# hermda02/dang

Measured on AMD Instinct MI355X. Metric: gibbs_iterations_per_sec, higher is better.
Workload: dtype f64

## Files before the change

### dang_amd/_lib.py

```python
import ctypes as C
import os

_HERE = os.path.dirname(os.path.abspath(__file__))
LIB_PATH = os.environ.get("DANGX_LIB") or os.path.join(_HERE, "lib", "libdangx.so")

MAX_BANDS, MAX_COMPS, MAX_IND, MAX_GROUP = 32, 16, 2, 8

POWERLAW, MBB, FREEFREE, LOGNORMAL, CMB, TCMB, TEMPLATE, MONOPOLE, HIFIT = 1, 2, 3, 4, 5, 6, 7, 8, 9
LNL_CHISQ, LNL_MARGINAL, LNL_PRIOR = 1, 2, 3
PRIOR_GAUSSIAN, PRIOR_UNIFORM, PRIOR_JEFFREYS = 1, 2, 3
ML_SAMPLE, ML_OPTIMIZE = 1, 2
FLAG_T, FLAG_Q, FLAG_U, FLAG_QU = 1, 2, 4, 8
SOLVER_DIRECT, SOLVER_CG = 0, 1
FLUCT_CORRECT, FLUCT_REFERENCE = 0, 1
COARSE_REFERENCE, COARSE_DEGRADED = 0, 1
COARSE_MODEL_CODES = {"reference": COARSE_REFERENCE, "degraded": COARSE_DEGRADED}
A2T, A2F, F2T = 0, 1, 2
UNIT_CODES = {"uK_RJ": 0, "uK_cmb": 1, "MJy/sr": 2}
K_AMP_DIRECT, K_INDEX_MH, K_SKY_CHISQ, K_REDUCE, K_CG_AX, K_CG_VEC, K_AMP_INDEX, K_MOMENTS = range(8)
KERNEL_NAMES = {K_AMP_DIRECT: "k_amp_direct", K_INDEX_MH: "k_index_mh", K_SKY_CHISQ: "k_sky_chisq",
                K_REDUCE: "k_reduce", K_CG_AX: "k_Ax", K_CG_VEC: "k_cg_vec", K_AMP_INDEX: "k_amp_index", K_MOMENTS: "k_moments"}
STAT_CODES = {"mean": 0, "std": 1}

TYPE_CODES = {"power-law": POWERLAW, "mbb": MBB, "freefree": FREEFREE, "lognormal": LOGNORMAL, "cmb": CMB, "T_cmb": TCMB,
              "template": TEMPLATE, "monopole": MONOPOLE, "hi_fit": HIFIT}
LNL_CODES = {"chisq": LNL_CHISQ, "marginal": LNL_MARGINAL, "prior": LNL_PRIOR}
PRIOR_CODES = {"gaussian": PRIOR_GAUSSIAN, "uniform": PRIOR_UNIFORM, "jeffreys": PRIOR_JEFFREYS}
ML_CODES = {"sample": ML_SAMPLE, "optimize": ML_OPTIMIZE}


class Dims(C.Structure):
    _fields_ = [("npix", C.c_int32), ("nmaps", C.c_int32), ("nbands", C.c_int32), ("ncomp", C.c_int32),
                ("pix0", C.c_int64), ("npix_global", C.c_int64), ("device", C.c_int32), ("reserved", C.c_int32)]


class CompDesc(C.Structure):
    _fields_ = [("type", C.c_int32), ("is_synch", C.c_int32), ("nindices", C.c_int32), ("cg_group", C.c_int32),
                ("sample_amplitude", C.c_int32), ("reserved", C.c_int32), ("nu_ref", C.c_double),
                ("lnl_type", C.c_int32 * MAX_IND), ("prior_type", C.c_int32 * MAX_IND),
                ("gauss_prior", (C.c_double * 2) * MAX_IND), ("uni_prior", (C.c_double * 2) * MAX_IND),
                ("step_size", C.c_double * MAX_IND)]


_P = C.c_void_p
_D = C.POINTER(C.c_double)
ALLREDUCE_FN = C.CFUNCTYPE(C.c_int, C.c_void_p, C.POINTER(C.c_double), C.c_int64)

SYMBOLS = {
    "dangx_create": (C.c_int, [C.POINTER(_P), C.POINTER(Dims)]),
    "dangx_destroy": (C.c_int, [_P]),
    "dangx_last_error": (C.c_char_p, [_P]),
    "dangx_version": (C.c_char_p, []),
    "dangx_set_stream": (C.c_int, [_P, _P]),
    "dangx_synchronize": (C.c_int, [_P]),
    "dangx_device_count": (C.c_int, [C.POINTER(C.c_int)]),
    "dangx_set_host_stride": (C.c_int, [_P, C.c_int64]),
    "dangx_set_allreduce": (C.c_int, [_P, _P, _P, C.c_int]),
    "dangx_index_sample_coarse": (C.c_int, [_P, C.c_int, C.c_int, C.c_int, C.c_int, C.c_int, C.c_uint64, C.c_uint64,
                                            C.c_int, C.c_int, C.POINTER(C.c_int64)]),
    "dangx_coarse_sizes": (C.c_int, [_P, C.c_int, C.c_int, C.POINTER(C.c_int64), C.POINTER(C.c_int64)]),
    "dangx_coarse_partials": (C.c_int, [_P, C.c_int, C.c_int, C.c_int, C.c_int, _P]),
    "dangx_coarse_chains": (C.c_int, [_P, C.c_int, C.c_int, C.c_int, C.c_int, C.c_int, C.c_uint64, C.c_uint64, C.c_int, C.c_int, _P, _P]),
    "dangx_coarse_writeback": (C.c_int, [_P, C.c_int, C.c_int, C.c_int, C.c_int, C.c_int, _P]),
    "dangx_set_coarse_model": (C.c_int, [_P, C.c_int, C.c_int, C.c_int]),
    "dangx_coarse_model_size": (C.c_int, [_P, C.c_int, C.c_int, C.c_int, C.POINTER(C.c_int64)]),
    "dangx_coarse_model_partials": (C.c_int, [_P, C.c_int, C.c_int, C.c_int, C.c_int, _P]),
    "dangx_coarse_model_finish": (C.c_int, [_P, C.c_int, C.c_int, C.c_int, C.c_int, _P]),
    "dangx_udgrade": (C.c_int, [_P, C.c_int, _P, C.c_int, _P, C.c_int]),
    "dangx_index_masked_sum": (C.c_int, [_P, C.c_int, C.c_int, C.c_int, C.POINTER(C.c_double), C.POINTER(C.c_int64)]),
    "dangx_index_plain_sum": (C.c_int, [_P, C.c_int, C.c_int, C.c_int, C.POINTER(C.c_double), C.POINTER(C.c_double)]),
    "dangx_unit_conversion": (C.c_int, [_P, C.c_int, C.c_int, _D]),
    "dangx_normalize_bandpass": (C.c_int, [_P, C.c_int, _P]),
    "dangx_convert_maps": (C.c_int, [_P, _P, _P, _P]),
    "dangx_set_band": (C.c_int, [_P, C.c_int, C.c_double, C.c_int, _P, _P]),
    "dangx_set_component": (C.c_int, [_P, C.c_int, C.POINTER(CompDesc)]),
    "dangx_set_tcmb": (C.c_int, [_P, C.c_double]),
    "dangx_set_calibration": (C.c_int, [_P, _P, _P]),
    "dangx_upload_data": (C.c_int, [_P, _P, _P, _P]),
    "dangx_adopt_device_data": (C.c_int, [_P, _P, _P, _P]),
    "dangx_put_amplitude": (C.c_int, [_P, C.c_int, _P]),
    "dangx_get_amplitude": (C.c_int, [_P, C.c_int, _P]),
    "dangx_put_indices": (C.c_int, [_P, C.c_int, _P]),
    "dangx_get_indices": (C.c_int, [_P, C.c_int, _P]),
    "dangx_set_template": (C.c_int, [_P, C.c_int, _P, _P, C.c_int]),
    "dangx_put_template_amplitudes": (C.c_int, [_P, C.c_int, _P]),
    "dangx_get_template_amplitudes": (C.c_int, [_P, C.c_int, _P]),
    "dangx_adopt_device_state": (C.c_int, [_P, C.c_int, _P, _P]),
    "dangx_amplitude_devptr": (_P, [_P, C.c_int]),
    "dangx_indices_devptr": (_P, [_P, C.c_int]),
    "dangx_amp_sample": (C.c_int, [_P, C.c_int, C.c_int, C.c_int, C.c_int, C.c_int, C.c_uint64, C.c_uint64,
                                   C.c_int, C.c_double, C.POINTER(C.c_int), C.POINTER(C.c_int64)]),
    "dangx_schur_info": (C.c_int, [_P, _D, C.POINTER(C.c_int)]),
    "dangx_amp_residual": (C.c_int, [_P, C.c_int, C.c_int, C.c_int, C.c_uint64, C.c_uint64, _D]),
    "dangx_index_sample": (C.c_int, [_P, C.c_int, C.c_int, C.c_int, C.c_int, C.c_int, C.c_uint64, C.c_uint64,
                                     C.POINTER(C.c_int64)]),
    "dangx_index_sample_pair": (C.c_int, [_P, C.c_int, C.c_int, C.c_int, C.c_int, C.c_int, C.c_uint64, C.c_uint64, C.c_uint64,
                                          C.POINTER(C.c_int64), C.POINTER(C.c_int64)]),
    "dangx_amp_index_sample": (C.c_int, [_P, C.c_int, C.c_int, C.c_int, C.c_int, C.c_int, C.c_uint64, C.c_uint64,
                                         C.c_int, C.c_double, C.c_int, C.c_int, C.c_int, C.c_int, C.c_uint64, C.c_uint64,
                                         C.POINTER(C.c_int), C.POINTER(C.c_int64), C.POINTER(C.c_int64)]),
    "dangx_plane_set_sample": (C.c_int, [_P, C.c_int, C.c_int, C.c_int, C.c_int, C.c_int, C.c_uint64, C.c_uint64, C.c_int, C.c_double,
                                         C.c_int, _P, _P, _P, C.c_int, C.c_uint64, C.POINTER(C.c_int), C.POINTER(C.c_int64), _P]),
    "dangx_plane_sweeps_sample": (C.c_int, [_P, C.c_int, C.c_int, _P, _P, _P, C.c_int, C.c_int, C.c_uint64, _P]),
    "dangx_sky_plane_set_sample": (C.c_int, [C.POINTER(_P), C.c_int, C.c_int, C.c_int, C.c_int, C.c_int, C.c_int, C.c_uint64, C.c_uint64, C.c_int,
                                             C.c_double, C.c_int, _P, _P, _P, C.c_int, C.c_uint64, C.POINTER(C.c_int), C.POINTER(C.c_int64), _P]),
    "dangx_sky_model_chisq": (C.c_int, [_P, C.c_int, C.c_int, _D, _P, _P, _P]),
    "dangx_sky_model_chisq_dev": (C.c_int, [_P, C.c_int, C.c_int, _P]),
    "dangx_chisq_cached": (C.c_int, [_P, C.c_int, C.c_int, C.c_int, _D]),
    "dangx_chisq_current": (C.c_int, [_P, C.c_int, C.c_int, _D]),
    "dangx_index_masked_sums": (C.c_int, [_P, C.c_int, _P, _P, _P, _P, _P]),
    "dangx_chisq_cached_dev": (C.c_int, [_P, C.c_int, C.c_int, C.c_int, _P]),
    "dangx_fullsky_prepare": (C.c_int, [_P, C.c_int, C.c_int]),
    "dangx_fullsky_prepare_coarse": (C.c_int, [_P, C.c_int, C.c_int, C.c_int, C.c_int]),
    "dangx_fullsky_sums": (C.c_int, [_P, C.c_int, _P, _P, C.c_int]),
    "dangx_fill_index": (C.c_int, [_P, C.c_int, C.c_int, C.c_int, C.c_double]),
    "dangx_gain_sums": (C.c_int, [_P, C.c_int, _P]),
    "dangx_peek_indices": (C.c_int, [_P, C.c_int, C.c_int, C.c_longlong, _P]),
    "dangx_fullsky_finish_coarse": (C.c_int, [_P, C.c_int, C.c_int, C.c_int, C.c_int, _P]),
    "dangx_fullsky_sample": (C.c_int, [C.POINTER(_P), C.c_int, C.c_int, C.c_int, C.c_int, C.c_int, C.c_int, C.c_uint64, C.c_uint64,
                                       C.c_int, C.c_int, C.POINTER(C.c_int32), _D, _D, C.POINTER(C.c_int64)]),
    "dangx_tune_step_size": (C.c_int, [C.POINTER(_P), C.c_int, C.c_int, C.c_int, C.c_int, C.c_int, C.c_uint64, C.c_uint64, _D,
                                       C.POINTER(C.c_uint32), C.POINTER(C.c_int32), _D]),
    "dangx_tune_perpixel": (C.c_int, [C.POINTER(_P), C.c_int, C.c_int, C.c_int, C.c_int, C.c_int, C.c_int, C.c_uint64, C.c_uint64,
                                      C.POINTER(C.c_int32), _D]),
    "dangx_fit_band_gain": (C.c_int, [C.POINTER(_P), C.c_int, C.c_int, C.c_int, C.c_uint64, C.c_uint64, _D]),
    "dangx_update_tcmb": (C.c_int, [C.POINTER(_P), C.c_int, C.c_int, _D]),
    "dangx_plan_fusion": (C.c_int, [_P, C.c_int, _P, _P, C.c_int, _P, _P, _P, _P, C.c_int, _P]),
    "dangx_sky_amp_sample": (C.c_int, [C.POINTER(_P), C.c_int, C.c_int, C.c_int, C.c_int, C.c_int, C.c_int, C.c_uint64, C.c_uint64,
                                       C.c_int, C.c_double, C.POINTER(C.c_int), C.POINTER(C.c_int64)]),
    "dangx_group_size": (C.c_int64, [_P, C.c_int, C.c_int]),
    "dangx_compute_rhs": (C.c_int, [_P, C.c_int, C.c_int, _P]),
    "dangx_compute_Ax": (C.c_int, [_P, C.c_int, C.c_int, _P, _P]),
    "dangx_compute_sample_vector": (C.c_int, [_P, C.c_int, C.c_int, _P, _P]),
    "dangx_eval_sed": (C.c_int, [_P, C.c_int, C.c_int, C.c_int, _P]),
    "dangx_rtc_kernels": (C.c_int, [_P, C.POINTER(C.c_int), C.c_char_p, C.c_int]),
    "dangx_rtc_compile": (C.c_int, [C.c_char_p, C.c_char_p, C.c_char_p, C.c_int]),
    "dangx_moments_begin": (C.c_int, [_P, _P]),
    "dangx_moments_accumulate": (C.c_int, [_P]),
    "dangx_moments_count": (C.c_int, [_P, C.POINTER(C.c_int64)]),
    "dangx_moments_get": (C.c_int, [_P, C.c_int, C.c_int, C.c_int, C.c_int, _P]),
    "dangx_moments_get_dev": (C.c_int, [_P, C.c_int, C.c_int, C.c_int, C.c_int, _P]),
    "dangx_moments_get_template": (C.c_int, [_P, C.c_int, C.c_int, C.c_int, _P]),
    "dangx_moments_end": (C.c_int, [_P]),
    "dangx_profile_enable": (C.c_int, [_P, C.c_int]),
    "dangx_profile_reset": (C.c_int, [_P]),
    "dangx_profile_get": (C.c_int, [_P, C.c_int, _D, C.POINTER(C.c_int64)]),
    "dangx_profile_get_planes": (C.c_int, [_P, C.c_int, C.c_int, _D, C.POINTER(C.c_int64)]),
}

_lib = None


def load():
    global _lib
    if _lib is not None:
        return _lib
    if not os.path.exists(LIB_PATH):
        raise RuntimeError(
            "libdangx.so is not built (%s). Run `python -c 'import __graft_entry__ as g; g.build()'`; "
            "there is no CPU fallback for the product path." % LIB_PATH)
    lib = C.CDLL(LIB_PATH)
    for name, (res, args) in SYMBOLS.items():
        fn = getattr(lib, name)
        fn.restype = res
        fn.argtypes = args
    _lib = lib
    return lib
```

### dang_amd/csrc/dangx_fused.hip

```cpp
#ifndef DX_NO_VCOEF
#define DX_VCOEF 1
#endif
#include "dx_host.h"
#include "dx_kern_fused.h"

static size_t fused_lds(int ng, int nb, int nv, int lanes) {
    return ((size_t)(TROWS * ng + 3) * nb + (size_t)nv * (nb / lanes + 2) * BLOCK) * sizeof(double);
}

#ifdef DX_REG_MODE
#define DX_CAT2(a, b) a##b
#define DX_CAT(a, b) DX_CAT2(a, b)
template <int NB, int NG, int LP>
static void launch_fused_case(dangx_ctx* ctx, const GroupArgs& ga, const FusedArgs& fa, const IndexArgs& a, int Sp, unsigned nblk,
                              unsigned long long* accp) {
    const size_t ldsz = fused_lds(NG, NB, fa.nv, LP);
    if (Sp == 2)
        hipLaunchKernelGGL((dxk::k_amp_index<DX_REG_MODE, 2, NB, NG, LP>), dim3(nblk), dim3(BLOCK), ldsz, ctx->stream, ctx->dm, ga, fa, a, ctx->counters, accp, ctx->partial);
    else
        hipLaunchKernelGGL((dxk::k_amp_index<DX_REG_MODE, 1, NB, NG, LP>), dim3(nblk), dim3(BLOCK), ldsz, ctx->stream, ctx->dm, ga, fa, a, ctx->counters, accp, ctx->partial);
}
bool DX_CAT(dx_launch_fused_mode, DX_REG_MODE)(dangx_ctx* ctx, const GroupArgs& ga, const FusedArgs& fa, const IndexArgs& a, int Sp,
                                              int lanes, unsigned nblk, unsigned long long* accp) {
    const int nb = ctx->hm.nbands;
    if (lanes == 1 && nb == 10 && ga.ng == 4) launch_fused_case<10, 4, 1>(ctx, ga, fa, a, Sp, nblk, accp);
    else if (lanes == 1 && nb == 10 && ga.ng == 3) launch_fused_case<10, 3, 1>(ctx, ga, fa, a, Sp, nblk, accp);
    else if (lanes == 1 && nb == 5 && ga.ng == 3) launch_fused_case<5, 3, 1>(ctx, ga, fa, a, Sp, nblk, accp);
    else if (lanes == 1 && nb == 3 && ga.ng == 2) launch_fused_case<3, 2, 1>(ctx, ga, fa, a, Sp, nblk, accp);
#if DX_REG_MODE == 1
    else if (lanes == 2 && nb == 20 && ga.ng == 6) launch_fused_case<20, 6, 2>(ctx, ga, fa, a, Sp, nblk, accp);
#endif
    else return false;
    return true;
}
#else
bool dx_launch_fused_mode1(dangx_ctx*, const GroupArgs&, const FusedArgs&, const IndexArgs&, int, int, unsigned, unsigned long long*);
bool dx_launch_fused_mode2(dangx_ctx*, const GroupArgs&, const FusedArgs&, const IndexArgs&, int, int, unsigned, unsigned long long*);
bool dx_launch_fused_mode3(dangx_ctx*, const GroupArgs&, const FusedArgs&, const IndexArgs&, int, int, unsigned, unsigned long long*);

static bool fused_builtin(int mode, int nb, int ng, int lanes) {
    if (lanes == 1) return (nb == 10 && (ng == 4 || ng == 3)) || (nb == 5 && ng == 3) || (nb == 3 && ng == 2);
    return mode == CH_POW && nb == 20 && ng == 6;
}

bool dx_fused_supported(int mode, int nb, int ng) {
    if (!(mode >= CH_POW && mode <= CH_MBB_T) || ng < 1 || ng > 6) return false;
    return fused_builtin(mode, nb, ng, 1) || fused_builtin(mode, nb, ng, 2) || dx_rtc_enabled();
}

static std::string fused_name(int mode, int Sp, int nb, int ng, int lanes) {
    return "dxk::k_amp_index<" + std::to_string(mode) + ", " + std::to_string(Sp) + ", " + std::to_string(nb) + ", " + std::to_string(ng) + ", " +
           std::to_string(lanes) + ">";
}

static bool fused_args(dangx_ctx* ctx, const GroupArgs& ga, const IndexArgs& a, FusedArgs& fa) {
    fa.nv = 0; fa.gself = -1;
    unsigned planes = 0;
    for (int k = a.s1; k <= a.s2; ++k) planes |= 1u << (k - 1);
    for (int g = 0; g < MAXG; ++g) { fa.vslot[g] = -1; fa.vcomp[g] = 0; fa.vtype[g] = 0; }
    for (int g = 0; g < ga.ng; ++g) {
        const Comp& c = ctx->hm.comp[ga.gc[g]];
        if (ga.gc[g] == a.comp) fa.gself = g;
        const unsigned cm = (unsigned)c.const_planes & planes;
        if (cm != 0 && cm != planes) return false;
        if (cm != planes) {
            if (c.type != DANGX_POWERLAW && c.type != DANGX_MBB && c.type != DANGX_FREEFREE && c.type != DANGX_LOGNORMAL) return false;
            fa.vcomp[fa.nv] = (signed char)g; fa.vtype[fa.nv] = (signed char)c.type;
            fa.vslot[g] = (signed char)fa.nv++;
        }
    }
    if (fa.gself < 0) return false;
    fa.cal = 0;
    if (a.s1 == 1)
        for (int j = 0; j < ctx->hm.nbands; ++j)
            if (ctx->hm.gain[j] != 1.0 || ctx->hm.offset[j] != 0.0) fa.cal = 1;
    return true;
}

int dx_fused_lanes(dangx_ctx* ctx, const GroupArgs& ga, const IndexArgs& a, int Sp) {
    if (!(a.mode >= CH_POW && a.mode <= CH_MBB_T) || ga.ng < 1 || ga.ng > 6) return 0;
    FusedArgs fa;
    if (!fused_args(ctx, ga, a, fa)) return 0;
    const int nb = ctx->hm.nbands, ng = ga.ng, cap = (Sp == 2) ? 10 : 16;
    int lanes = 0;
    if (nb <= cap && fused_lds(ng, nb, fa.nv, 1) <= 80u * 1024u) lanes = 1;
    else if (nb % 2 == 0 && nb / 2 <= cap && dx_mh_reg_lanes(nb, Sp) == 2 && fused_lds(ng, nb, fa.nv, 2) <= 80u * 1024u) lanes = 2;
    if (!lanes) return 0;
    if (fused_builtin(a.mode, nb, ng, lanes)) return lanes;
    return dx_rtc_get(ctx, "dx_kern_fused.h", fused_name(a.mode, Sp, nb, ng, lanes)) ? lanes : 0;
}

bool dx_launch_fused(dangx_ctx* ctx, const GroupArgs& ga, const IndexArgs& a, int Sp, int lanes, unsigned nblk, unsigned long long* accp) {
    FusedArgs fa;
    if (lanes < 1 || !fused_args(ctx, ga, a, fa)) return false;
    bool done = false;
    switch (a.mode) {
    case CH_POW: done = dx_launch_fused_mode1(ctx, ga, fa, a, Sp, lanes, nblk, accp); break;
    case CH_MBB_BETA: done = dx_launch_fused_mode2(ctx, ga, fa, a, Sp, lanes, nblk, accp); break;
    case CH_MBB_T: done = dx_launch_fused_mode3(ctx, ga, fa, a, Sp, lanes, nblk, accp); break;
    default: return false;
    }
    if (done) return true;
    const int nb = ctx->hm.nbands, ng = ga.ng;
    hipFunction_t fn = dx_rtc_get(ctx, "dx_kern_fused.h", fused_name(a.mode, Sp, nb, ng, lanes));
    if (!fn) return false;
    const Model* dm = ctx->dm;
    GroupArgs gg = ga;
    IndexArgs aa = a;
    unsigned long long* bad = ctx->counters;
    double* part = ctx->partial;
    void* args[] = {&dm, &gg, &fa, &aa, &bad, &accp, &part};
    return dx_rtc_launch(ctx, fn, nblk, fused_lds(ng, nb, fa.nv, lanes), args) == 0;
}
#endif
```

### dang_amd/csrc/dangx_planeset.hip

```cpp
#ifndef DX_NO_VCOEF
#define DX_VCOEF 1
#endif
#include "dx_host.h"
#include "dx_kern_planeset.h"

static size_t planeset_lds(int ng, int nb, int nv, int lanes, int Sp) {
    const int rows = nv > Sp ? nv : Sp;
    return ((size_t)(TROWS * ng + 3) * nb + (size_t)rows * (nb / lanes) * BLOCK) * sizeof(double);
}

static void item_codes(const SweepList& sl, int code[4]) {
    for (int q = 0; q < 4; ++q) code[q] = (q < sl.n) ? sl.s[q].mode + 8 * sl.s[q].pair : 0;
}
static std::string planeset_name(int Sp, int nb, int ng, int lanes, int solve, const SweepList& sl, int bp) {
    int c[4];
    item_codes(sl, c);
    std::string s = "dxk::k_plane_set<" + std::to_string(Sp) + ", " + std::to_string(nb) + ", " + std::to_string(ng) + ", " + std::to_string(lanes) +
                    ", " + std::to_string(solve);
    for (int q = 0; q < 4; ++q) s += ", " + std::to_string(c[q]);
    return s + ", " + std::to_string(bp) + ">";
}

static int planeset_bp(dangx_ctx* ctx) {
    for (int j = 0; j < ctx->hm.nbands; ++j)
        if (ctx->hm.band[j].n != 0) return 1;
    return 0;
}

static bool planeset_builtin(int nb, int ng, int lanes, int solve, const SweepList& sl) {
    int c[4];
    item_codes(sl, c);
    if (nb == 20 && ng == 6 && lanes == 2) return solve && c[0] == CH_POW && c[1] == CH_MBB_BETA + 8 && c[2] == CH_LOGN_NUP && c[3] == 0;
    if (lanes == 1 && nb == 10 && ng == 4 && solve && sl.n == 0) return true;
    if (lanes == 1 && ((nb == 10 && ng == 4) || (solve && ((nb == 5 && ng == 3) || (nb == 3 && ng == 2)))))
        return c[0] == CH_POW && c[1] == CH_MBB_BETA + 8 && c[2] == 0 && c[3] == 0;
    return false;
}

template <int NB, int NG, int LP, int SOLVE, int C0, int C1, int C2>
static void launch_builtin(dangx_ctx* ctx, const GroupArgs& ga, const FusedArgs& fa, const SweepList& sl, int Sp, unsigned nblk, size_t ldsz,
                           unsigned long long* accp) {
    if (Sp == 2)
        hipLaunchKernelGGL((dxk::k_plane_set<2, NB, NG, LP, SOLVE, C0, C1, C2, 0>), dim3(nblk), dim3(BLOCK), ldsz, ctx->stream, ctx->dm, ga, fa, sl, ctx->counters, accp, ctx->partial);
    else
        hipLaunchKernelGGL((dxk::k_plane_set<1, NB, NG, LP, SOLVE, C0, C1, C2, 0>), dim3(nblk), dim3(BLOCK), ldsz, ctx->stream, ctx->dm, ga, fa, sl, ctx->counters, accp, ctx->partial);
}

static bool planeset_args(dangx_ctx* ctx, const GroupArgs& ga, const SweepList& sl, FusedArgs& fa) {
    fa.nv = 0; fa.gself = -1;
    unsigned planes = 0;
    for (int k = sl.s1; k <= sl.s2; ++k) planes |= 1u << (k - 1);
    for (int g = 0; g < MAXG; ++g) { fa.vslot[g] = -1; fa.vcomp[g] = 0; fa.vtype[g] = 0; }
    for (int g = 0; g < ga.ng; ++g) {
        const int l = ga.gc[g];
        const Comp& c = ctx->hm.comp[l];
        const unsigned cm = (unsigned)c.const_planes & planes;
        if (cm != 0 && cm != planes) return false;
        if (cm != planes) {
            if (c.type != DANGX_POWERLAW && c.type != DANGX_MBB && c.type != DANGX_FREEFREE && c.type != DANGX_LOGNORMAL) return false;
            if (sl.s2 > sl.s1 && (ctx->qu_equal[l] & ((1u << c.nind) - 1u)) != ((1u << c.nind) - 1u)) return false;
            fa.vcomp[fa.nv] = (signed char)g; fa.vtype[fa.nv] = (signed char)c.type;
            fa.vslot[g] = (signed char)fa.nv++;
        }
    }
    fa.cal = 0;
    if (sl.s1 == 1)
        for (int j = 0; j < ctx->hm.nbands; ++j)
            if (ctx->hm.gain[j] != 1.0 || ctx->hm.offset[j] != 0.0) fa.cal = 1;
    return true;
}

int dx_planeset_lanes(dangx_ctx* ctx, const GroupArgs& ga, const SweepList& sl, int solve) {
    static const bool enabled = [] { const char* e = getenv("DANGX_PLANESET"); return !(e && e[0] == '0'); }();
    static const bool small_too = [] { const char* e = getenv("DANGX_PLANESET"); return !(e && e[0] == 'p'); }();
    if (!enabled || sl.n < 0 || sl.n > 4 || (sl.n == 0 && !solve) || ga.ng < 1 || ga.ng > 6) return 0;
    static const int cap2 = [] { const char* e = getenv("DANGX_PS_CAP2"); return e ? atoi(e) : 13; }();
    const int nb = ctx->hm.nbands, Sp = sl.s2 - sl.s1 + 1, cap = (Sp == 2) ? cap2 : 16;
    for (int q = 0; q < sl.n; ++q) {
        const int m = sl.s[q].mode;
        if (m < CH_POW || m > CH_LOGN_W) return 0;
        if (sl.s[q].pair && !(m == CH_MBB_BETA || m == CH_LOGN_NUP)) return 0;
    }
    FusedArgs fa;
    if (!planeset_args(ctx, ga, sl, fa)) return 0;
    if (solve && fa.cal && ga.nuc > 0) return 0;
    const int bp = planeset_bp(ctx);
    if (bp) {
        for (int q = 0; q < sl.n; ++q)
            if (sl.s[q].mode > CH_MBB_T) return 0;
        if (!(small_too && nb <= cap && planeset_lds(ga.ng, nb, fa.nv, 1, Sp) <= 80u * 1024u)) return 0;
        return dx_rtc_get(ctx, "dx_kern_planeset.h", planeset_name(Sp, nb, ga.ng, 1, solve, sl, 1)) ? 1 : 0;
    }
    int lanes = 0;
    if (small_too && nb <= cap && planeset_lds(ga.ng, nb, fa.nv, 1, Sp) <= 80u * 1024u) lanes = 1;
    else if (nb > 12 && nb % 2 == 0 && nb / 2 <= cap && planeset_lds(ga.ng, nb, fa.nv, 2, Sp) <= 80u * 1024u) lanes = 2;
    if (!lanes) return 0;
    if (planeset_builtin(nb, ga.ng, lanes, solve, sl)) return lanes;
    return dx_rtc_get(ctx, "dx_kern_planeset.h", planeset_name(Sp, nb, ga.ng, lanes, solve, sl, 0)) ? lanes : 0;
}

bool dx_launch_planeset(dangx_ctx* ctx, const GroupArgs& ga, const SweepList& sl, int lanes, int solve, unsigned nblk, unsigned long long* accp) {
    FusedArgs fa;
    if (lanes < 1 || lanes > 2 || !planeset_args(ctx, ga, sl, fa)) return false;
    const int nb = ctx->hm.nbands, ng = ga.ng, Sp = sl.s2 - sl.s1 + 1;
    const size_t ldsz = planeset_lds(ng, nb, fa.nv, lanes, Sp);
    const int bp = planeset_bp(ctx);
    if (!bp && planeset_builtin(nb, ng, lanes, solve, sl)) {
        if (nb == 20) launch_builtin<20, 6, 2, 1, CH_POW, CH_MBB_BETA + 8, CH_LOGN_NUP>(ctx, ga, fa, sl, Sp, nblk, ldsz, accp);
        else if (nb == 10 && sl.n == 0) launch_builtin<10, 4, 1, 1, 0, 0, 0>(ctx, ga, fa, sl, Sp, nblk, ldsz, accp);
        else if (nb == 10 && !solve) launch_builtin<10, 4, 1, 0, CH_POW, CH_MBB_BETA + 8, 0>(ctx, ga, fa, sl, Sp, nblk, ldsz, accp);
        else if (nb == 10) launch_builtin<10, 4, 1, 1, CH_POW, CH_MBB_BETA + 8, 0>(ctx, ga, fa, sl, Sp, nblk, ldsz, accp);
        else if (nb == 5) launch_builtin<5, 3, 1, 1, CH_POW, CH_MBB_BETA + 8, 0>(ctx, ga, fa, sl, Sp, nblk, ldsz, accp);
        else launch_builtin<3, 2, 1, 1, CH_POW, CH_MBB_BETA + 8, 0>(ctx, ga, fa, sl, Sp, nblk, ldsz, accp);
        return true;
    }
    hipFunction_t fn = dx_rtc_get(ctx, "dx_kern_planeset.h", planeset_name(Sp, nb, ng, lanes, solve, sl, bp));
    if (!fn) return false;
    const Model* dm = ctx->dm;
    GroupArgs gg = ga;
    SweepList ss = sl;
    unsigned long long* bad = ctx->counters;
    double* part = ctx->partial;
    void* args[] = {&dm, &gg, &fa, &ss, &bad, &accp, &part};
    return dx_rtc_launch(ctx, fn, nblk, ldsz, args) == 0;
}

#ifdef DX_LNL_DIAG
extern "C" int dangx_lnl_diag(unsigned long long* out) {
    if (hipMemcpyFromSymbol(out, HIP_SYMBOL(g_lnl_diag), 2 * sizeof(unsigned long long)) != hipSuccess) return 1;
    const unsigned long long z[2] = {0ull, 0ull};
    return hipMemcpyToSymbol(HIP_SYMBOL(g_lnl_diag), z, sizeof(z)) == hipSuccess ? 0 : 1;
}
#endif
```

### dang_amd/csrc/dangx_rtc.hip

```cpp
#include "dx_host.h"

#include <hip/hiprtc.h>
#include <sys/stat.h>
#include <unistd.h>

#include <fstream>
#include <sstream>
#include <string>
#include <vector>

#include "dx_rtc_embed.h"

namespace {

unsigned long long fnv1a(unsigned long long h, const char* p, size_t n) {
    for (size_t i = 0; i < n; ++i) { h ^= (unsigned char)p[i]; h *= 1099511628211ull; }
    return h;
}

std::string cache_dir() {
    const char* e = getenv("DANGX_CACHE_DIR");
    std::string d;
    if (e && e[0]) d = e;
    else if ((e = getenv("HOME")) && e[0]) d = std::string(e) + "/.cache/dangx";
    else d = "/tmp/dangx-cache-" + std::to_string((long)getuid());
    std::string acc;
    for (size_t i = 0; i <= d.size(); ++i)
        if (i == d.size() || (d[i] == '/' && i > 0)) { acc = d.substr(0, i); (void)mkdir(acc.c_str(), 0700); }
    struct stat st;
    if (lstat(d.c_str(), &st) != 0 || !S_ISDIR(st.st_mode) || st.st_uid != getuid() || (st.st_mode & (S_IWGRP | S_IWOTH)) != 0) {
        static bool told = false;
        if (!told && getenv("DANGX_RTC_VERBOSE")) fprintf(stderr, "[dangx] %s is not a private directory of this user: no disk cache\n", d.c_str());
        told = true;
        return std::string();
    }
    return d;
}

bool read_file(const std::string& path, std::string& out) {
    std::ifstream f(path, std::ios::binary);
    if (!f) return false;
    std::ostringstream ss;
    ss << f.rdbuf();
    out = ss.str();
    return !out.empty();
}
void write_file_atomic(const std::string& path, const std::string& data) {
    const std::string tmp = path + ".tmp" + std::to_string((long)getpid());
    {
        std::ofstream f(tmp, std::ios::binary);
        if (!f) return;
        f.write(data.data(), (std::streamsize)data.size());
        if (!f) { (void)unlink(tmp.c_str()); return; }
    }
    if (rename(tmp.c_str(), path.c_str()) != 0) (void)unlink(tmp.c_str());
}

const char* const kOptions[] = {"--offload-arch=gfx950", "-O3", "-std=c++17"};
constexpr int kNumOptions = 3;

std::vector<std::string> extra_options() {
    std::vector<std::string> out;
    const char* e = getenv("DANGX_RTC_DEFS");
    if (!e) return out;
    std::istringstream ss(e);
    std::string w;
    while (ss >> w) out.push_back(w);
    return out;
}

int compile(dangx_ctx* ctx, const char* header, const std::string& name_expr, std::string& code, std::string& lowered) {
    const std::string src = std::string("#define DX_VCOEF 1\n#include \"") + header + "\"\n";
    hiprtcProgram prog;
    if (hiprtcCreateProgram(&prog, src.c_str(), "dangx_rtc_unit.hip", DX_RTC_NFILES, dx_rtc_texts, dx_rtc_names) != HIPRTC_SUCCESS)
        return fail(ctx, "hiprtcCreateProgram failed");
    int rc = 0;
    if (hiprtcAddNameExpression(prog, name_expr.c_str()) != HIPRTC_SUCCESS) rc = fail(ctx, "hiprtcAddNameExpression failed for " + name_expr);
    const std::vector<std::string> extra = extra_options();
    std::vector<const char*> opts(kOptions, kOptions + kNumOptions);
    for (const auto& o : extra) opts.push_back(o.c_str());
    if (!rc && hiprtcCompileProgram(prog, (int)opts.size(), opts.data()) != HIPRTC_SUCCESS) {
        size_t n = 0;
        (void)hiprtcGetProgramLogSize(prog, &n);
        std::string log(n, '\0');
        if (n) (void)hiprtcGetProgramLog(prog, &log[0]);
        rc = fail(ctx, "run-time compilation of " + name_expr + " failed:\n" + log.substr(0, 4000));
    }
    if (!rc) {
        const char* low = nullptr;
        size_t n = 0;
        if (hiprtcGetLoweredName(prog, name_expr.c_str(), &low) != HIPRTC_SUCCESS || !low) rc = fail(ctx, "no lowered name for " + name_expr);
        else lowered = low;
        if (!rc && (hiprtcGetCodeSize(prog, &n) != HIPRTC_SUCCESS || n == 0)) rc = fail(ctx, "empty code object for " + name_expr);
        if (!rc) { code.resize(n); if (hiprtcGetCode(prog, &code[0]) != HIPRTC_SUCCESS) rc = fail(ctx, "hiprtcGetCode failed"); }
    }
    (void)hiprtcDestroyProgram(&prog);
    return rc;
}

}

bool dx_rtc_enabled() {
    static const bool on = [] { const char* e = getenv("DANGX_RTC"); return !(e && e[0] == '0'); }();
    return on;
}

hipFunction_t dx_rtc_get(dangx_ctx* ctx, const char* header, const std::string& name_expr) {
    if (!dx_rtc_enabled()) return nullptr;
    for (const auto& e : ctx->rtc_fns)
        if (e.first == name_expr) return e.second;
    for (const auto& n : ctx->rtc_failed)
        if (n == name_expr) return nullptr;
    unsigned long long h = 1469598103934665603ull;
    auto mix = [&](const char* p, size_t n) {
        const unsigned long long len = n;
        h = fnv1a(h, reinterpret_cast<const char*>(&len), sizeof(len));
        h = fnv1a(h, p, n);
    };
    for (int i = 0; i < DX_RTC_NFILES; ++i) { mix(dx_rtc_names[i], strlen(dx_rtc_names[i])); mix(dx_rtc_texts[i], strlen(dx_rtc_texts[i])); }
    for (int i = 0; i < kNumOptions; ++i) mix(kOptions[i], strlen(kOptions[i]));
    for (const auto& o : extra_options()) mix(o.data(), o.size());
    int maj = 0, min = 0;
    (void)hiprtcVersion(&maj, &min);
    hipDeviceProp_t prop;
    std::string arch = "?";
    if (hipGetDeviceProperties(&prop, ctx->device) == hipSuccess) arch = prop.gcnArchName;
    const std::string tagv = std::string(header) + "|" + name_expr + "|" + std::to_string(maj) + "." + std::to_string(min) + "|" + arch;
    mix(tagv.data(), tagv.size());
    char hex[32];
    snprintf(hex, sizeof(hex), "%016llx", h);
    const std::string dir = cache_dir();
    const std::string base = dir + "/k_" + hex;
    std::string code, lowered;
    const bool cached = !dir.empty() && read_file(base + ".hsaco", code) && read_file(base + ".sym", lowered);
    if (!cached) {
        if (getenv("DANGX_RTC_VERBOSE")) fprintf(stderr, "[dangx] specialising %s (hiprtc)\n", name_expr.c_str());
        if (compile(ctx, header, name_expr, code, lowered)) { ctx->rtc_failed.push_back(name_expr); return nullptr; }
        if (!dir.empty()) {
            write_file_atomic(base + ".hsaco", code);
            write_file_atomic(base + ".sym", lowered);
        }
    }
    (void)hipSetDevice(ctx->device);
    hipModule_t mod = nullptr;
    hipFunction_t fn = nullptr;
    if (hipModuleLoadData(&mod, code.data()) != hipSuccess || hipModuleGetFunction(&fn, mod, lowered.c_str()) != hipSuccess) {
        if (mod) (void)hipModuleUnload(mod);
        if (cached) {
            (void)unlink((base + ".hsaco").c_str());
            (void)unlink((base + ".sym").c_str());
            return dx_rtc_get(ctx, header, name_expr);
        }
        ctx->err = "could not load the specialised kernel " + name_expr;
        ctx->rtc_failed.push_back(name_expr);
        return nullptr;
    }
    ctx->rtc_mods.push_back(mod);
    ctx->rtc_fns.emplace_back(name_expr, fn);
    return fn;
}

int dx_rtc_launch(dangx_ctx* ctx, hipFunction_t fn, unsigned nblk, size_t lds, void** args) {
    HIPCHK(ctx, hipModuleLaunchKernel(fn, nblk, 1, 1, BLOCK, 1, 1, (unsigned)lds, ctx->stream, args, nullptr));
    return 0;
}

void dx_rtc_release(dangx_ctx* ctx) {
    for (hipModule_t m : ctx->rtc_mods) (void)hipModuleUnload(m);
    ctx->rtc_mods.clear();
    ctx->rtc_fns.clear();
}

extern "C" int dangx_rtc_compile(const char* header, const char* name_expr, char* log, int log_len) {
    if (!header || !name_expr) return 1;
    dangx_ctx tmp;
    std::string code, lowered;
    const int rc = compile(&tmp, header, name_expr, code, lowered);
    if (log && log_len > 0) snprintf(log, (size_t)log_len, "%s", rc ? tmp.err.c_str() : lowered.c_str());
    return rc;
}

extern "C" int dangx_rtc_kernels(dangx_ctx* ctx, int* n, char* names, int names_len) {
    if (!ctx || !n) return 1;
    *n = (int)ctx->rtc_fns.size();
    if (names && names_len > 0) {
        std::string all;
        for (const auto& e : ctx->rtc_fns) all += e.first + "\n";
        snprintf(names, (size_t)names_len, "%s", all.c_str());
    }
    return 0;
}
```

### dang_amd/csrc/dx_chain.h

```cpp
#pragma once
#include "dx_args.h"


template <bool V> struct BoolTag { static constexpr bool value = V; };

#ifdef DX_CHAIN_LIBEXP
#define CEXP(x) exp(x)
#define CEXPS(x) exp(x)
#define CEXP1(x) exp(x)
#else
#define CEXP(x) exp_nr(x)
#define CEXPS(x) exp_sat(x)
#define CEXP1(x) exp_nr_v(x)
#endif
#ifdef DX_CHAIN_IEEEDIV
#define CDIV(a, b) ((a) / (b))
#else
#define CDIV(a, b) ((a) * fast_rcp(b))
#endif

#ifndef DX_CHAIN_UNSCALED
#define DX_CHAIN_SCALED 1
#endif
#ifndef DX_CHAIN_PAIR_RNG
#define DX_CHAIN_PAIR_RNG 1
#endif

namespace {

__device__ __forceinline__ bool mh_accept(double diff, double u3) {
#if defined(DX_ACCEPT_FULL) || defined(DX_CHAIN_LIBEXP)
    return (diff >= 0.0) || (CEXP1(diff) > u3);
#else
    const float e = __builtin_amdgcn_exp2f((float)diff * 0x1.715476p+0f);
    const float uf = (float)u3;
    bool acc = (diff >= 0.0) || (e > uf * 0x1.001p+0f);
    const bool unsure = !(acc || e < uf * 0x1.ffep-1f);
    if (__builtin_amdgcn_ballot_w64(unsure) != 0ull) {
        if (unsure) acc = CEXP1(diff) > u3;
    }
    return acc;
#endif
}

__device__ __forceinline__ bool mh_certain(double dlo, double dhi, double u3, bool& acc) {
    const float uf = (float)u3;
    const float elo = __builtin_amdgcn_exp2f((float)dlo * 0x1.715476p+0f);
    const float ehi = __builtin_amdgcn_exp2f((float)dhi * 0x1.715476p+0f);
    acc = (dlo >= 0.0) || (elo > uf * 0x1.001p+0f);
    return acc || ((dhi < 0.0) && (ehi < uf * 0x1.ffep-1f));
}


#ifdef DX_LNL_DIAG
__device__ unsigned long long g_lnl_diag[2];
__device__ __forceinline__ void lnl_diag_count(int k) {
    if (__lane_id() == __builtin_ctzll(__builtin_amdgcn_ballot_w64(true))) atomicAdd(&g_lnl_diag[k], 1ull);
}
#endif

template <int LP>
struct BandPick {
    int half;
    __device__ __forceinline__ double operator()(const double* arr, int j, int nbh) const {
        if (LP == 1) return arr[j];
        const double a = arr[j], b = arr[nbh + j];
        return half ? b : a;
    }
    __device__ __forceinline__ double nu_c(const Model& M, int j, int nbh) const {
        if (LP == 1) return M.band[j].nu_c;
        const double a = M.band[j].nu_c, b = M.band[nbh + j].nu_c;
        return half ? b : a;
    }
};

template <int MODE, int SP, int NB, int LP, bool KT = false, bool BP = false>
struct RegChain {
    static constexpr bool kBP = BP;
    double D[SP][NB], F[NB], ISr[SP][NB];
    double bpa, bpb;
    double K1[(LP > 1 && !KT) ? NB : 1], K2[(LP > 1 && !KT) ? NB : 1];
    const double *kt1, *kt2;
    double amp[SP];

    __device__ __forceinline__ double is(int kk, int j) const { return ISr[kk][j]; }
    __device__ __forceinline__ void set_is(int kk, int j, double v) { ISr[kk][j] = v; }
    __device__ __forceinline__ double k1(const Model& M, const Comp& c, int j) const {
        if (KT) return kt1[j];
        if (LP > 1) return K1[j];
        return (MODE == CH_MBB_T) ? M.band[j].nu_c : (MODE == CH_LOGN_NUP) ? c.lnu9[j] : c.lnr[j];
    }
    __device__ __forceinline__ double k2(const Comp& c, int j) const { return KT ? kt2[j] : (LP > 1) ? K2[j] : c.cst[j]; }
    __device__ __forceinline__ void set_kt(const double* tab, int nbands, int ng, int g, int jb) {
        kt1 = tab + ((MODE == CH_MBB_T) ? TROWS * ng : (MODE == CH_LOGN_NUP) ? TROWS * g + 2 : TROWS * g) * nbands + jb;
        kt2 = tab + (TROWS * g + 1) * nbands + jb;
    }
    __device__ __forceinline__ void set_k(const Model& M, const Comp& c, const BandPick<LP>& pick) {
        if (LP > 1 && !KT) {
#pragma unroll
            for (int j = 0; j < NB; ++j) {
                K1[j] = (MODE == CH_MBB_T) ? pick.nu_c(M, j, NB) : (MODE == CH_LOGN_NUP) ? pick(c.lnu9, j, NB) : pick(c.lnr, j, NB);
                K2[j] = (MODE == CH_LOGN_NUP || MODE == CH_LOGN_W) ? pick(c.cst, j, NB) : 0.0;
            }
        }
    }

    template <bool BATCH, int OP = 0>
    __device__ __forceinline__ double lnl(const Model& M, const Comp& c, double th, double other, double& acc0, double& acc1) {
        double s0 = 0.0, s1 = 0.0;
        if (MODE == CH_POW) s0 = th;
        else if (MODE == CH_MBB_BETA) s0 = th + 1.0;
        else if (MODE == CH_MBB_T) { s0 = mbb_z(th); s1 = CEXP(s0 * c.nu_ref) - 1.0; }
        else if (MODE == CH_LOGN_NUP) { s0 = log_pos(th); s1 = other; }
        else s1 = th;
        acc0 = 0.0; acc1 = 0.0;
#ifdef DX_CHAIN_IEEEDIV
        const double rs1 = 1.0 / s1;
#else
        const double rs1 = (MODE == CH_LOGN_NUP || MODE == CH_LOGN_W) ? fast_rcp(s1) : 0.0;
#endif
        constexpr int TT = BP ? 1 : (NB % 5 == 0) ? 5 : (NB % 4 == 0) ? 4 : (NB % 3 == 0) ? 3 : 1;
        static_assert(!BP || (LP == 1 && (MODE == CH_POW || MODE == CH_MBB_BETA || MODE == CH_MBB_T)), "bandpass chains: one lane, power law / mbb");
#pragma unroll
        for (int j0 = 0; j0 < NB; j0 += TT) {
            double s[TT];
            if (BP && M.band[j0].n != 0) {
                const Band& b = M.band[j0];
                const kptr nu = as_const(M.bp_nu0 + b.off);
                const kptr tau = as_const(M.bp_tau0 + b.off);
                const kptr lnr = as_const(c.bp_lnr + b.off);
                const int n = b.n;
                double sj = 0.0;
                if (MODE == CH_POW) {
#pragma unroll 4
                    for (int q = 0; q < n; ++q) sj = sj + tau[q] * CEXP(s0 * lnr[q]);
                } else if (MODE == CH_MBB_BETA) {
#pragma unroll 4
                    for (int q = 0; q < n; ++q) sj = sj + (tau[q] * bpb) * fast_rcp(CEXP(bpa * nu[q]) - 1.0) * CEXP(s0 * lnr[q]);
                } else {
#pragma unroll 4
                    for (int q = 0; q < n; ++q) sj = sj + (tau[q] * s1) * fast_rcp(CEXP(s0 * nu[q]) - 1.0) * CEXP(bpa * lnr[q]);
                }
                s[0] = sj;
            } else
            if (MODE == CH_MBB_T && TT > 1 && BATCH) {
                double den[TT], pre[TT];
#pragma unroll
                for (int t = 0; t < TT; ++t) den[t] = CEXP(s0 * k1(M, c, j0 + t)) - 1.0;
                pre[0] = den[0];
#pragma unroll
                for (int t = 1; t < TT; ++t) pre[t] = pre[t - 1] * den[t];
                double inv = s1 * fast_rcp(pre[TT - 1]);
#pragma unroll
                for (int t = TT - 1; t > 0; --t) {
                    s[t] = (inv * pre[t - 1]) * F[j0 + t];
                    inv *= den[t];
                }
                s[0] = inv * F[j0];
            } else
#pragma unroll
            for (int t = 0; t < TT; ++t) {
                const int j = j0 + t;
                if (MODE == CH_LOGN_NUP) {
                    const double l = (k1(M, c, j) - s0) * rs1;
                    s[t] = CEXPS(-0.5 * (l * l)) * k2(c, j);
                } else if (MODE == CH_LOGN_W) {
                    const double l = F[j] * rs1;
                    s[t] = CEXPS(-0.5 * (l * l)) * k2(c, j);
                } else {
                    const double e = CEXP(s0 * k1(M, c, j));
                    if (MODE == CH_POW) s[t] = e;
                    else if (MODE == CH_MBB_BETA) s[t] = F[j] * e;
                    else s[t] = CDIV(s1, e - 1.0) * F[j];
                }
            }
#pragma unroll
            for (int t = 0; t < TT; ++t) {
                const int j = j0 + t;
#ifdef DX_CHAIN_SCALED
                if (OP == 1) {
                    const double r0 = D[0][j];
                    D[0][j] = fma(is(0, j), s[t], r0);
                    acc0 = fma(r0, r0, acc0);
                    if (SP == 2) {
                        const double r1 = D[SP - 1][j];
                        D[SP - 1][j] = fma(is(SP - 1, j), s[t], r1);
                        acc1 = fma(r1, r1, acc1);
                    }
                } else if (OP == 2) {
                    const double r0 = fma(-is(0, j), s[t], D[0][j]);
                    D[0][j] = r0;
                    acc0 = fma(r0, r0, acc0);
                    if (SP == 2) {
                        const double r1 = fma(-is(SP - 1, j), s[t], D[SP - 1][j]);
                        D[SP - 1][j] = r1;
                        acc1 = fma(r1, r1, acc1);
                    }
                } else {
                const double r0 = fma(-is(0, j), s[t], D[0][j]);
                acc0 = fma(r0, r0, acc0);
                if (SP == 2) {
                    const double r1 = fma(-is(SP - 1, j), s[t], D[SP - 1][j]);
                    acc1 = fma(r1, r1, acc1);
                }
                }
#else
                const double r0 = (D[0][j] - amp[0] * s[t]) * is(0, j);
                acc0 = acc0 - 0.5 * (r0 * r0);
                if (SP == 2) {
                    const double r1 = (D[SP - 1][j] - amp[SP - 1] * s[t]) * is(SP - 1, j);
                    acc1 = acc1 - 0.5 * (r1 * r1);
                }
#endif
            }
        }
        if (LP > 1) {
            acc0 += __shfl_xor(acc0, 1, 64);
            if (SP == 2) acc1 += __shfl_xor(acc1, 1, 64);
        }
#ifdef DX_CHAIN_SCALED
        acc0 *= -0.5; acc1 *= -0.5;
#endif
        return acc0 + acc1;
    }

    __device__ __forceinline__ double lnl_cheap(const Model& M, const Comp& c, double th) {
        double s0 = 0.0, s1 = 0.0;
        if (MODE == CH_POW) s0 = th;
        else if (MODE == CH_MBB_BETA) s0 = th + 1.0;
        else { s0 = mbb_z(th); s1 = CEXP(s0 * c.nu_ref) - 1.0; }
        const double s0l = s0 * 0x1.71547652b82fep+0;
        double acc0 = 0.0, acc1 = 0.0;
#pragma unroll
        for (int j = 0; j < NB; ++j) {
            const float e = __builtin_amdgcn_exp2f((float)(s0l * k1(M, c, j)));
            double s;
            if (MODE == CH_POW) s = (double)e;
            else if (MODE == CH_MBB_BETA) s = F[j] * (double)e;
            else s = (s1 * F[j]) * (double)__builtin_amdgcn_rcpf(e - 1.0f);
            const double r0 = fma(-is(0, j), s, D[0][j]);
            acc0 = fma(r0, r0, acc0);
            if (SP == 2) {
                const double r1 = fma(-is(SP - 1, j), s, D[SP - 1][j]);
                acc1 = fma(r1, r1, acc1);
            }
        }
        double a = acc0 + acc1;
        if (LP > 1) a += __shfl_xor(a, 1, 64);
        return a;
    }

    __device__ __forceinline__ bool cheap_bound(const Model& M, const Comp& c, double lo, double hi, double a_start,
                                                double& wA, double& wG) {
        double G = 0.0, emax = 0.0, kmax = 0.0;
        double smax, zmin = 0.0;
        if (MODE == CH_POW) smax = fmax(fabs(lo), fabs(hi));
        else if (MODE == CH_MBB_BETA) smax = fmax(fabs(lo + 1.0), fabs(hi + 1.0));
        else { smax = mbb_z(lo); zmin = mbb_z(hi); }
#pragma unroll
        for (int j = 0; j < NB; ++j) {
            const double k = fabs(k1(M, c, j));
            kmax = fmax(kmax, k);
            double e;
            if (MODE == CH_MBB_T) e = (1.0 + smax * k) * 0x1p-24 + (2.0 + (double)__builtin_amdgcn_rcpf((float)(zmin * k))) * 0x1p-22;
            else e = (smax * k) * 0x1p-24 + 0x1p-22;
            e = e * (1.0 + 0x1p-8) + 0x1p-46;
            emax = fmax(emax, e);
#pragma unroll
            for (int kk = 0; kk < SP; ++kk) { const double t = e * D[kk][j]; G = fma(t, t, G); }
        }
        if (LP > 1) { G += __shfl_xor(G, 1, 64); emax = fmax(emax, __shfl_xor(emax, 1, 64)); kmax = fmax(kmax, __shfl_xor(kmax, 1, 64)); }
        const double lam = fmax(sqrt(G * fast_rcp(fmax(a_start, 0x1p-900))), 0x1p-400);
        wA = 0.5 * ((2.0 * emax * (1.0 + emax) + lam) * (1.0 + 0x1p-40) + 0x1p-40);
        wG = 0.5 * ((G * fast_rcp(lam) + 2.0 * G) * (1.0 + 0x1p-40) + 0x1p-1000);
        const bool range = smax * kmax * 0x1.71547652b82fep+0 <= 125.0;
        return (MODE == CH_MBB_T) ? (range && lo > 0.0 && zmin > 0.0) : range;
    }
    __device__ __forceinline__ void scale() {
#ifdef DX_CHAIN_SCALED
#pragma unroll
        for (int kk = 0; kk < SP; ++kk)
#pragma unroll
            for (int j = 0; j < NB; ++j) { D[kk][j] *= ISr[kk][j]; ISr[kk][j] *= amp[kk]; }
#endif
    }
};

template <int NB, int LP>
__device__ __forceinline__ void subtract_other(const Model& M, const Comp& c2, int k, double amp2, double t0, double t1,
                                               double (&Dk)[NB], const BandPick<LP>& pick) {
    if ((c2.const_planes >> (k - 1)) & 1) {
#pragma unroll
        for (int j = 0; j < NB; ++j) Dk[j] -= amp2 * pick(c2.csed[k - 1], j, NB);
        return;
    }
    const Prep pr = sed_prep(c2, t0, t1);
    switch (c2.type) {
    case DANGX_POWERLAW:
#pragma unroll
        for (int j = 0; j < NB; ++j) Dk[j] -= amp2 * CEXP(pr.p0 * pick(c2.lnr, j, NB));
        break;
    case DANGX_MBB:
#pragma unroll
        for (int j = 0; j < NB; ++j) Dk[j] -= amp2 * (CDIV(pr.p2, CEXP(pr.p1 * pick.nu_c(M, j, NB)) - 1.0) * CEXP(pr.p0 * pick(c2.lnr, j, NB)));
        break;
    case DANGX_FREEFREE:
#pragma unroll
        for (int j = 0; j < NB; ++j) Dk[j] -= amp2 * (ff_gaunt(pick(c2.lnu9, j, NB), pr.p0) / pr.p1 * pick(c2.cst, j, NB));
        break;
    case DANGX_LOGNORMAL: {
        const double rp1 = fast_rcp(pr.p1);
#pragma unroll
        for (int j = 0; j < NB; ++j) {
            const double l2 = (pick(c2.lnu9, j, NB) - pr.p2) * rp1;
            Dk[j] -= amp2 * (CEXPS(-0.5 * (l2 * l2)) * pick(c2.cst, j, NB));
        }
        break;
    }
    default:
#pragma unroll
        for (int j = 0; j < NB; ++j) Dk[j] -= amp2 * pick(c2.cst, j, NB);
        break;
    }
}

template <int NB, int LP>
__device__ __forceinline__ void subtract_other_pair(const Model& M, const Comp& c2, double ampa, double ampb, double t0, double t1,
                                                    double (&Da)[NB], double (&Db)[NB], const BandPick<LP>& pick) {
    const Prep pr = sed_prep(c2, t0, t1);
    switch (c2.type) {
    case DANGX_POWERLAW:
#pragma unroll
        for (int j = 0; j < NB; ++j) { const double s = CEXP(pr.p0 * pick(c2.lnr, j, NB)); Da[j] -= ampa * s; Db[j] -= ampb * s; }
        break;
    case DANGX_MBB:
#pragma unroll
        for (int j = 0; j < NB; ++j) {
            const double s = CDIV(pr.p2, CEXP(pr.p1 * pick.nu_c(M, j, NB)) - 1.0) * CEXP(pr.p0 * pick(c2.lnr, j, NB));
            Da[j] -= ampa * s; Db[j] -= ampb * s;
        }
        break;
    case DANGX_FREEFREE:
#pragma unroll
        for (int j = 0; j < NB; ++j) {
            const double s = ff_gaunt(pick(c2.lnu9, j, NB), pr.p0) / pr.p1 * pick(c2.cst, j, NB);
            Da[j] -= ampa * s; Db[j] -= ampb * s;
        }
        break;
    case DANGX_LOGNORMAL: {
        const double rp1 = fast_rcp(pr.p1);
#pragma unroll
        for (int j = 0; j < NB; ++j) {
            const double l2 = (pick(c2.lnu9, j, NB) - pr.p2) * rp1;
            const double s = CEXPS(-0.5 * (l2 * l2)) * pick(c2.cst, j, NB);
            Da[j] -= ampa * s; Db[j] -= ampb * s;
        }
        break;
    }
    default:
#pragma unroll
        for (int j = 0; j < NB; ++j) { const double s = pick(c2.cst, j, NB); Da[j] -= ampa * s; Db[j] -= ampb * s; }
        break;
    }
}

template <int MODE, int SP, int NB, int LP, bool SCALE = true, bool ADD = false, bool SUB = false, class RC>
__device__ __forceinline__ unsigned long long chain_finish(const Model& M, const IndexArgs& a, const Comp& c, RC& R,
                                                           const BandPick<LP>& pick, double sample0, double sample1, int i, int half,
                                                           double chi[4], double* final_value = nullptr,
                                                           const double* acc_in = nullptr, double* acc_out = nullptr) {
    const int npix = M.npix;
    double* out = c.idx + ((long long)a.nind * M.nmaps) * npix + i;
    const bool first = (a.nind == 0);
    if (SCALE) R.scale();
    if (MODE == CH_MBB_BETA) {
        const double z = mbb_z(sample1);
        const double A = CEXP(z * c.nu_ref) - 1.0;
#pragma unroll
        for (int j = 0; j < NB; ++j) R.F[j] = CDIV(A, CEXP(z * pick.nu_c(M, j, NB)) - 1.0);
        if (RC::kBP) { R.bpa = z; R.bpb = A; }
    } else if (MODE == CH_MBB_T) {
#pragma unroll
        for (int j = 0; j < NB; ++j) R.F[j] = CEXP((sample0 + 1.0) * pick(c.lnr, j, NB));
        if (RC::kBP) R.bpa = sample0 + 1.0;
    } else if (MODE == CH_LOGN_W) {
        {
            const double lp = log_pos(sample0);
#pragma unroll
            for (int j = 0; j < NB; ++j) R.F[j] = pick(c.lnu9, j, NB) - lp;
        }
    }
    const double other = first ? sample1 : sample0;
    const unsigned long long gpix = (unsigned long long)(M.pix0 + i);
    const int q = a.nind;
    const bool gauss = c.prior_type[q] == DANGX_PRIOR_GAUSSIAN;
    const double pmean = c.gauss[q][0], pstd = c.gauss[q][1], lgden = c.lgden[q];
    const double inv2v = 1.0 / (2 * (pstd * pstd));
    auto prior = [&](double v) -> double {
        if (!gauss) return 0.0;
#ifdef DX_CHAIN_IEEEDIV
        const double arg = ((v - pmean) * (v - pmean)) / (2 * (pstd * pstd));
#else
        const double arg = ((v - pmean) * (v - pmean)) * inv2v;
#endif
        return (arg > 745.0) ? -INFINITY : -arg - lgden;
    };
    unsigned long long nacc = 0;
    double cur = first ? sample0 : sample1;
    double a0, a1, c0, c1;
    const double step = c.step[q], lo = c.uni[q][0], hi = c.uni[q][1];
    const bool ml_opt = (a.ml_mode == DANGX_ML_OPTIMIZE);
#if defined(DX_LNL_EXACT) || !defined(DX_CHAIN_SCALED)
    constexpr bool kCert = false;
#else
    constexpr bool kCert = !RC::kBP && (MODE == CH_POW || MODE == CH_MBB_BETA || MODE == CH_MBB_T);
#endif
    auto chain = [&](auto batch_tag) {
        constexpr bool B = decltype(batch_tag)::value;
        double lnl;
        if (acc_in) { a0 = acc_in[0]; a1 = acc_in[1]; lnl = a0 + a1; }
        else lnl = R.template lnl<B, ADD ? 1 : 0>(M, c, cur, other, a0, a1);
        chi[0] = -2.0 * a0; chi[1] = -2.0 * a1;
        double lnl_old = lnl + prior(cur);
        bool cert = false, old_exact = true, sums_exact = true;
        double wA = 0.0, wG = 0.0, wold = 0.0;
        if (kCert) {
            const bool ok = R.cheap_bound(M, c, lo, hi, -2.0 * lnl, wA, wG) && !ml_opt;
            cert = __builtin_amdgcn_ballot_w64(!ok) == 0ull;
        }
        auto mh_step = [&](double prop, double u3) {
            if (prop < lo || prop > hi) return;
            if constexpr (!kCert) {
                lnl = R.template lnl<B>(M, c, prop, other, c0, c1);
                const double lnl_new = lnl + prior(prop);
                const double diff = lnl_new - lnl_old;
                const bool acc = ml_opt ? (diff > 0.0) : mh_accept(diff, u3);
                if (acc) { cur = prop; lnl_old = lnl_new; a0 = c0; a1 = c1; ++nacc; }
            } else {
                const double pp = prior(prop);
                bool acc = false, und = true;
                double lc = 0.0, wc = 0.0;
                if (cert) {
                    const double A = R.lnl_cheap(M, c, prop);
                    lc = -0.5 * A;
                    wc = fma(wA, A, wG);
                    const double dc = (lc + pp) - lnl_old;
                    const double W = (wc + wold) * (1.0 + 0x1p-40) + 0x1p-49 * ((fabs(lc) + fabs(pp)) + fabs(lnl_old));
                    und = !mh_certain(dc - W, dc + W, u3, acc);
#ifdef DX_LNL_DIAG
                    lnl_diag_count(0);
                    if (__builtin_amdgcn_ballot_w64(und) != 0ull) lnl_diag_count(1);
#endif
                }
                if (__builtin_amdgcn_ballot_w64(und) != 0ull) {
                    if (und) {
                        bool again = !old_exact;
#pragma unroll 1
                        for (;;) {
                            const double l = R.template lnl<B>(M, c, again ? cur : prop, other, c0, c1);
                            if (!again) { lnl = l; break; }
                            lnl_old = l + prior(cur);
                            again = false;
                        }
                        const double lnl_new = lnl + pp;
                        const double diff = lnl_new - lnl_old;
                        acc = ml_opt ? (diff > 0.0) : mh_accept(diff, u3);
                        if (acc) { lnl_old = lnl_new; a0 = c0; a1 = c1; }
                        old_exact = true;
                        wold = 0.0;
                    }
                }
                if (acc) {
                    cur = prop;
                    ++nacc;
                    sums_exact = und;
                    if (!und) { lnl_old = lc + pp; wold = wc; old_exact = false; }
                }
            }
        };
        if (LP == 1 || DX_CHAIN_PAIR_RNG == 0) {
            for (int l = 1; l <= a.nsample; ++l) {
                double u1, u2, u3;
                uniform3(a.seed, a.stream, gpix, (uint32_t)l, u1, u2, u3);
                mh_step(cur + rand_normal(0.0, step, u1, u2), u3);
            }
        } else {
            for (int l = 1; l <= a.nsample; l += 2) {
                double u1, u2, u3;
                uniform3(a.seed, a.stream, gpix, (uint32_t)(l + half), u1, u2, u3);
                const double g = rand_normal(0.0, step, u1, u2);
                const double go = __shfl_xor(g, 1, 64), uo = __shfl_xor(u3, 1, 64);
                mh_step(cur + (half == 0 ? g : go), half == 0 ? u3 : uo);
                if (l + 1 <= a.nsample) mh_step(cur + (half == 0 ? go : g), half == 0 ? uo : u3);
            }
        }
        if (SUB) {
            double s0_, s1_;
            (void)R.template lnl<B, 2>(M, c, cur, other, s0_, s1_);
            if (!sums_exact) { a0 = s0_; a1 = s1_; }
        } else if (kCert) {
            if (__builtin_amdgcn_ballot_w64(!sums_exact) != 0ull) {
                if (!sums_exact) (void)R.template lnl<B>(M, c, cur, other, a0, a1);
            }
        }
    };
#ifdef DX_CHAIN_NO_BATCH_RCP
    chain(BoolTag<false>{});
#else
    if (MODE == CH_MBB_T && !RC::kBP) {
        const double tmin = fmin(lo, cur);
#ifdef DX_BATCH_ALWAYS
        chain(BoolTag<true>{});
#elif defined(DX_BATCH_LANEWISE)
        if (tmin > 0.0 && mbb_z(tmin) * M.mbb_batch_z < 1.0) chain(BoolTag<true>{});
        else chain(BoolTag<false>{});
#else
        const bool unsafe = !(tmin > 0.0 && mbb_z(tmin) * M.mbb_batch_z < 1.0);
        if (__builtin_amdgcn_ballot_w64(unsafe) == 0ull) chain(BoolTag<true>{});
        else chain(BoolTag<false>{});
#endif
    } else {
        chain(BoolTag<false>{});
    }
#endif
    if (final_value) *final_value = cur;
    if (acc_out) { acc_out[0] = a0; acc_out[1] = a1; }
    if (half != 0) {
        chi[0] = chi[1] = 0.0;
        return 0ull;
    }
#pragma unroll
    for (int kk = 0; kk < SP; ++kk) out[(long long)(a.s1 + kk - 1) * npix] = cur;
    chi[2] = -2.0 * a0; chi[3] = -2.0 * a1;
    return nacc;
}

template <int MODE, int SP, int NB, int LP>
__device__ __forceinline__ void index_chain_stage(const Model& M, const IndexArgs& a, const Comp& c, RegChain<MODE, SP, NB, LP>& R,
                                                  const BandPick<LP>& pick, int i, double& sample0, double& sample1) {
    const int npix = M.npix;
    const int jb = pick.half * NB;
    R.set_k(M, c, pick);
    load_theta(M, c, i, a.s1, sample0, sample1);
    const long long bstride = (long long)M.nmaps * npix;
#pragma unroll
    for (int kk = 0; kk < SP; ++kk) {
        const int k = a.s1 + kk;
        R.amp[kk] = c.amp[(long long)(k - 1) * npix + i];
        const double* sigp = M.sig + (long long)(k - 1) * npix + i;
        const double* rmsp = M.rms + (long long)(k - 1) * npix + i;
        double rv[NB];
#pragma unroll
        for (int j = 0; j < NB; ++j) {
            R.D[kk][j] = sigp[(jb + j) * bstride];
            rv[j] = rmsp[(jb + j) * bstride];
        }
#pragma unroll
        for (int j = 0; j < NB; ++j) {
            if (k == 1) R.D[kk][j] = (R.D[kk][j] - pick(M.offset, j, NB)) / pick(M.gain, j, NB);
            R.set_is(kk, j, CDIV(1.0, rv[j]));
        }
    }
    {
        unsigned om = a.others;
        double na[SP], nt0[SP], nt1[SP];
        auto fetch = [&](int l) {
            const Comp& c2 = M.comp[l];
#pragma unroll
            for (int kk = 0; kk < SP; ++kk) {
                na[kk] = c2.amp[(long long)(a.s1 + kk - 1) * npix + i];
                nt0[kk] = nt1[kk] = 0.0;
                if (!((c2.const_planes >> (a.s1 + kk - 1)) & 1)) load_theta(M, c2, i, a.s1 + kk, nt0[kk], nt1[kk]);
            }
        };
        int l = om ? __builtin_ctz(om) : -1;
        if (l >= 0) fetch(l);
        while (l >= 0) {
            const Comp& c2 = M.comp[l];
            double ca[SP], ct0[SP], ct1[SP];
#pragma unroll
            for (int kk = 0; kk < SP; ++kk) { ca[kk] = na[kk]; ct0[kk] = nt0[kk]; ct1[kk] = nt1[kk]; }
            om &= om - 1;
            const int ln = om ? __builtin_ctz(om) : -1;
            if (ln >= 0) fetch(ln);
            const unsigned cp = (c2.const_planes >> (a.s1 - 1)) & 3u;
            if (SP == 2 && cp == 0 && ct0[0] == ct0[SP - 1] && ct1[0] == ct1[SP - 1]) {
                subtract_other_pair<NB, LP>(M, c2, ca[0], ca[SP - 1], ct0[0], ct1[0], R.D[0], R.D[SP - 1], pick);
            } else {
#pragma unroll
                for (int kk = 0; kk < SP; ++kk) subtract_other<NB, LP>(M, c2, a.s1 + kk, ca[kk], ct0[kk], ct1[kk], R.D[kk], pick);
            }
            l = ln;
        }
    }
}

template <int MODE, int SP, int NB, int LP>
__device__ __forceinline__ unsigned long long index_chain_reg(const Model& M, const IndexArgs& a, int i, int half, double chi[4]) {
    const int npix = M.npix;
    const Comp& c = M.comp[a.comp];
    double* out = c.idx + ((long long)a.nind * M.nmaps) * npix + i;
    if (is_masked(M.mask[i])) {
        if (half == 0) {
#pragma unroll
            for (int kk = 0; kk < SP; ++kk) out[(long long)(a.s1 + kk - 1) * npix] = 0.0;
        }
        return 0ull;
    }
    const BandPick<LP> pick = {half};
    RegChain<MODE, SP, NB, LP> R;
    double sample0, sample1;
    index_chain_stage<MODE, SP, NB, LP>(M, a, c, R, pick, i, sample0, sample1);
    return chain_finish<MODE, SP, NB, LP>(M, a, c, R, pick, sample0, sample1, i, half, chi);
}

template <int MODEA, int MODEB, int SP, int NB, int LP>
__device__ __forceinline__ void index_chain_pair(const Model& M, const IndexArgs& a, const IndexArgs& b, int i, int half, double chi[4],
                                                 unsigned long long& nacc_a, unsigned long long& nacc_b) {
    const int npix = M.npix;
    const Comp& c = M.comp[a.comp];
    nacc_a = nacc_b = 0ull;
    if (is_masked(M.mask[i])) {
        if (half == 0) {
#pragma unroll
            for (int kk = 0; kk < SP; ++kk) {
                c.idx[((long long)a.nind * M.nmaps + (a.s1 + kk - 1)) * npix + i] = 0.0;
                c.idx[((long long)b.nind * M.nmaps + (a.s1 + kk - 1)) * npix + i] = 0.0;
            }
        }
        return;
    }
    const BandPick<LP> pick = {half};
    RegChain<MODEA, SP, NB, LP> RA;
    double sample0, sample1;
    index_chain_stage<MODEA, SP, NB, LP>(M, a, c, RA, pick, i, sample0, sample1);
    double chia[4] = {0.0, 0.0, 0.0, 0.0}, chib[4] = {0.0, 0.0, 0.0, 0.0}, va;
    nacc_a = chain_finish<MODEA, SP, NB, LP>(M, a, c, RA, pick, sample0, sample1, i, half, chia, &va);
    RegChain<MODEB, SP, NB, LP> RB;
    RB.set_k(M, c, pick);
#pragma unroll
    for (int kk = 0; kk < SP; ++kk) {
        RB.amp[kk] = RA.amp[kk];
#pragma unroll
        for (int j = 0; j < NB; ++j) { RB.D[kk][j] = RA.D[kk][j]; RB.ISr[kk][j] = RA.ISr[kk][j]; }
    }
    if (a.nind == 0) sample0 = va; else sample1 = va;
    nacc_b = chain_finish<MODEB, SP, NB, LP, false>(M, b, c, RB, pick, sample0, sample1, i, half, chib);
    chi[0] = chia[0]; chi[1] = chia[1]; chi[2] = chib[2]; chi[3] = chib[3];
}

}
```

### dang_amd/csrc/dx_host.h

```cpp
#pragma once
#include <hip/hip_runtime.h>

#include <algorithm>
#include <cmath>
#include <cstdio>
#include <cstdlib>
#include <cstring>
#include <string>
#include <vector>

#include "../../include/dangx.h"
#include "dx_args.h"

struct DxMoments;

struct dangx_ctx {
    dangx_dims dims{};
    int device = 0;
    hipStream_t stream = nullptr;
    std::string err;
    Model hm{};
    Model* dm = nullptr;
    bool dirty = true;
    bool comp_set[MAXC] = {};
    bool band_set[MAXB] = {};
    dangx_comp_desc desc[MAXC] = {};
    double *sig = nullptr, *rms = nullptr, *mask = nullptr;
    bool own_data = false;
    double* amp[MAXC] = {};
    double* idx[MAXC] = {};
    bool own_amp[MAXC] = {};
    bool own_idx[MAXC] = {};
    unsigned plane_nz[MAXC] = {};
    double* tmpl[MAXC] = {};
    int corr_mask[MAXC] = {}, nfit[MAXC] = {};
    double tamp[MAXC][3][MAXB] = {};
    unsigned tmpl_nz[MAXC] = {};
    unsigned tmpl_one[MAXC] = {};
    unsigned idx_const[MAXC] = {};
    unsigned qu_equal[MAXC] = {};
    double idx_val[MAXC][3][MAXI] = {};
    bool idxsum_ok[MAXC][MAXI][3] = {};
    double idxsum[MAXC][MAXI][3] = {};
    long long idxcnt[MAXC][MAXI][3] = {};
    bool idx_ext[MAXC] = {};
    bool idxsum_dev[MAXC][MAXI][3] = {};
    long long mask_count = -1;
    std::vector<double> bp_nu0, bp_tau0;
    double *d_bp_nu0 = nullptr, *d_bp_tau0 = nullptr, *d_bp_lnr = nullptr;
    bool bp_dirty = true;
    double* partial = nullptr;
    long long partial_cap = 0;
    double* scalars = nullptr;
    double* chi_cache = nullptr;
    double chi_host[3] = {0.0, 0.0, 0.0};
    static constexpr int CHI_RING = 8;
    struct ChiPend { double* buf = nullptr; long long cap = 0, nblk = 0; int s1 = 0, s2 = 0, wb = 0, ns = 0; int slot[DX_MAX_IDXSUM] = {}; } chi_pend[CHI_RING];
    int chi_npend = 0;
    double* chi_stage = nullptr;
    bool chi_before_valid[3] = {}, chi_after_valid[3] = {}, touched_since_amp[3] = {};
    unsigned long long* counters = nullptr;
    long long host_stride = 0;
    dangx_allreduce_fn allreduce = nullptr;
    void* allreduce_user = nullptr;
    bool is_root = true;
    double* work[6] = {};
    double* fs_data = nullptr;
    long long fs_cap = 0;
    int fs_comp = -1, fs_s1 = 0, fs_s2 = 0;
    unsigned fs_others = 0;
    bool fs_lazy = false;
    long long fs_npc = 0;
    double* rows_out = nullptr;
    int hp_nside = 0, hp_cnside = 0;
    int *hp_n2r_f = nullptr, *hp_r2n_f = nullptr, *hp_n2r_c = nullptr, *hp_r2n_c = nullptr;
    double *cs_data = nullptr, *cs_rms = nullptr, *cs_mask = nullptr, *cs_index = nullptr;
    long long cs_cap = 0;
    struct CsKept { int s1 = 0, s2 = 0, nside = 0, sample_nside = 0; long long gen = -1, cap = 0, capm = 0, stamp = 0; double *rms = nullptr, *mask = nullptr; };
    CsKept cs_kept[2];
    long long data_gen = 0, cs_stamp = 0;
    double* cs_part = nullptr;
    long long cs_part_cap = 0;
    unsigned cm_degraded[MAXC] = {};
    double* cs_model = nullptr;
    long long cm_cap = 0;
    double* cm_part = nullptr;
    long long cm_part_cap = 0;
    bool cm_ok = false;
    int cm_comp = -1, cm_s1 = 0, cm_s2 = 0, cm_nside = 0, cm_cnside = 0;
    const double* fs_camp = nullptr;
    long long work_cap = 0;
    double schur_resid = 0.0, schur_backward = 0.0;
    bool defer_amp = false, have_pending = false;
    bool pair_on = false, pair_done = false;
    unsigned long long pair_stream = 0;
    GroupArgs pending{};
    long long pending_SN = 0;
    int schur_refine = 0;
    std::vector<std::pair<std::string, hipFunction_t>> rtc_fns;
    std::vector<hipModule_t> rtc_mods;
    std::vector<std::string> rtc_failed;
    bool prof = false;
    struct Ev { hipEvent_t a, b; int kid, planes; };
    std::vector<Ev> events;
    double prof_ms[DANGX_K_COUNT] = {};
    long long prof_n[DANGX_K_COUNT] = {};
    double prof_ms_pl[DANGX_K_COUNT][3] = {};
    long long prof_n_pl[DANGX_K_COUNT][3] = {};
    DxMoments* mom = nullptr;
};

struct DxRoctx {
    int (*push)(const char*) = nullptr;
    int (*pop)() = nullptr;
    DxRoctx();
};
const DxRoctx& dx_roctx();
struct DxRange {
    bool on;
    explicit DxRange(const char* name) : on(dx_roctx().push != nullptr) { if (on) (void)dx_roctx().push(name); }
    ~DxRange() { if (on) (void)dx_roctx().pop(); }
    DxRange(const DxRange&) = delete;
    DxRange& operator=(const DxRange&) = delete;
};
const char* dx_kernel_family(int kid);

#define HIPCHK(ctx, call)                                                                         \
    do {                                                                                          \
        hipError_t e_ = (call);                                                                   \
        if (e_ != hipSuccess) {                                                                   \
            (ctx)->err = std::string(#call) + ": " + hipGetErrorString(e_);                       \
            return 1;                                                                             \
        }                                                                                         \
    } while (0)

inline void invalidate_chi(dangx_ctx* ctx) {
    ctx->cm_ok = false;
    for (int k = 0; k < 3; ++k) ctx->chi_before_valid[k] = ctx->chi_after_valid[k] = false;
    if (ctx->chi_npend) {
        for (int l = 0; l < MAXC; ++l)
            for (int q = 0; q < MAXI; ++q) for (int k = 0; k < 3; ++k) ctx->idxsum_dev[l][q][k] = false;
    }
    ctx->chi_npend = 0;
}

inline void idx_written(dangx_ctx* ctx, int comp) {
    ctx->cm_ok = false;
    for (int l = 0; l < MAXC; ++l)
        if (comp < 0 || l == comp)
            for (int q = 0; q < MAXI; ++q) for (int k = 0; k < 3; ++k) ctx->idxsum_ok[l][q][k] = ctx->idxsum_dev[l][q][k] = false;
    if (comp < 0) ctx->mask_count = -1;
}
inline void qu_written(dangx_ctx* ctx, int comp, int nind, int map_n) {
    if (map_n == -1) ctx->qu_equal[comp] |= 1u << nind;
    else if (map_n == 2 || map_n == 3) ctx->qu_equal[comp] &= ~(1u << nind);
}
inline int idx_slot(int comp, int nind, int plane) { return 6 + (comp * MAXI + nind) * 3 + (plane - 1); }
constexpr int CHI_CACHE_DOUBLES = 6 + MAXC * MAXI * 3;

inline int fail(dangx_ctx* ctx, const std::string& msg) {
    ctx->err = msg;
    return 1;
}

struct Timed {
    dangx_ctx* ctx;
    dangx_ctx::Ev ev{};
    bool on;
    DxRange range;
    Timed(dangx_ctx* c, int kid, int planes = 0) : ctx(c), on(c->prof), range(dx_kernel_family(kid)) {
        if (!on) return;
        ev.kid = kid; ev.planes = (planes >= 0 && planes <= 2) ? planes : 0;
        (void)hipEventCreate(&ev.a);
        (void)hipEventCreate(&ev.b);
        (void)hipEventRecord(ev.a, ctx->stream);
    }
    ~Timed() {
        if (!on) return;
        (void)hipEventRecord(ev.b, ctx->stream);
        ctx->events.push_back(ev);
    }
};


inline int ensure_partial(dangx_ctx* ctx, long long n) {
    if (n <= ctx->partial_cap) return 0;
    if (ctx->partial) (void)hipFree(ctx->partial);
    HIPCHK(ctx, hipMalloc(&ctx->partial, sizeof(double) * (size_t)n));
    ctx->partial_cap = n;
    return 0;
}

inline int flag_planes_h(int flag) { return (flag & DANGX_FLAG_QU) ? 2 : 1; }

inline unsigned nblocks(long long n, int bs = BLOCK) { return (unsigned)((n + bs - 1) / bs); }

void dx_reduce_rows_to(dangx_ctx* ctx, const double* partial, unsigned nblk, int rows, double* out_dev);
constexpr int DX_RSTAGE = 128;
void dx_reduce_two_stage(dangx_ctx* ctx, const double* partial, long long n, double* stage, double* out_dev);

int sync_model(dangx_ctx* ctx);
int prof_collect(dangx_ctx* ctx);
void dx_moments_free(dangx_ctx* ctx);
int ensure_work(dangx_ctx* ctx, long long n);
int ensure_state(dangx_ctx* ctx, int comp);
int check_comp(dangx_ctx* ctx, int comp);
int copy_planes(dangx_ctx* ctx, void* dst, const void* src, size_t planes, bool to_device);
int make_group(dangx_ctx* ctx, int group, int flag, GroupArgs& a);
int dx_set_chi_after(dangx_ctx* ctx, int k, double chi);
int chi_flush(dangx_ctx* ctx);
int chi_next(dangx_ctx* ctx, long long nblk, double** buf);
int reduce_to_host(dangx_ctx* ctx, long long nblk, double* out);
int rank_sum(dangx_ctx* ctx, double* buf, int64_t n);
int device_cg(dangx_ctx* ctx, const GroupArgs& a, int i_max, double converge, int* iters);
extern "C" int dx_fullsky_prepare_lazy(dangx_ctx* ctx, int comp, int map_n);
extern "C" int dx_fullsky_coarse_model(dangx_ctx* ctx, int comp, int nind);
double dx_host_band_sed(dangx_ctx* ctx, int comp, int j, double t0, double t1);
int device_schur(dangx_ctx* const* cs, int nc, const GroupArgs* as, const long long* SNs, int64_t* n_not_spd, int* nullity, int* defer = nullptr);
inline int map_planes(dangx_ctx* ctx, int map_n, int& s1, int& s2) {
    if (map_n == -1) { s1 = 2; s2 = 3; }
    else if (map_n >= 1 && map_n <= 3) { s1 = s2 = map_n; }
    else return fail(ctx, "There is something wrong with the poltype flag (map_n must be 1,2,3 or -1)");
    if (s2 > ctx->dims.nmaps) return fail(ctx, "map_n exceeds nmaps");
    return 0;
}

bool dx_rtc_enabled();
hipFunction_t dx_rtc_get(dangx_ctx* ctx, const char* header, const std::string& name_expr);
int dx_rtc_launch(dangx_ctx* ctx, hipFunction_t fn, unsigned nblk, size_t lds, void** args);
void dx_rtc_release(dangx_ctx* ctx);

int dx_launch_amp(dangx_ctx* ctx, const GroupArgs& a, long long SN);
int dx_launch_amp_reg(dangx_ctx* ctx, const GroupArgs& a, long long SN);
int dx_launch_chisq_reg(dangx_ctx* ctx, int k, double* partial);
int dx_launch_amp_reg_templates(dangx_ctx* ctx, const GroupArgs& a, long long SN);
struct SchurArgs;
int dx_launch_schur_resid_reg(dangx_ctx* ctx, const GroupArgs& a, const SchurArgs& sa, long long SN, double* rows_dev);
int dx_launch_schur_pass1_reg(dangx_ctx* ctx, const GroupArgs& a, const SchurArgs& sa, long long SN, double* rows_dev);
int dx_launch_rhs(dangx_ctx* ctx, const GroupArgs& a, long long SN, double* b);
int dx_launch_Ax(dangx_ctx* ctx, const GroupArgs& a, long long SN, const double* x, double* res, double* part);
int dx_launch_sample_vector(dangx_ctx* ctx, const GroupArgs& a, long long SN, const double* eta, double* res);
constexpr int DX_MAX_ROWS = 32;
struct SchurArgs {
    int nrows;
    unsigned char rt[DX_MAX_ROWS], rj[DX_MAX_ROWS];
    signed char ftarget[DX_MAX_ROWS];
    signed char bslot[MAXB];
    int nslots;
};
int dx_launch_schur_pass1(dangx_ctx* ctx, const GroupArgs& a, const SchurArgs& sa, long long SN, double* rows_dev);
int dx_launch_schur_pass2(dangx_ctx* ctx, const GroupArgs& a, long long SN);
int dx_launch_schur_resid(dangx_ctx* ctx, const GroupArgs& a, const SchurArgs& sa, long long SN, double* rows_dev);
int dx_launch_rhs_mixed(dangx_ctx* ctx, const GroupArgs& a, long long SN, double* b);
int dx_launch_Ax_mixed(dangx_ctx* ctx, const GroupArgs& a, long long SN, const double* x, double* res);
int dx_launch_sv_mixed(dangx_ctx* ctx, const GroupArgs& a, long long SN, const double* eta, double* res);
void dx_launch_mh_lds(dangx_ctx* ctx, const IndexArgs& a, bool fast, int Sp, unsigned nblk, int bs, size_t lds, unsigned long long* accp);
bool dx_mh_reg_supported(dangx_ctx* ctx, int mode, int nb, int Sp);
bool dx_mh_pair_supported(int mode_a, int mode_b, int nb, int Sp);
bool dx_launch_mh_pair(dangx_ctx* ctx, const IndexArgs& a, const IndexArgs& b, int Sp, unsigned nblk, unsigned long long* accp);
bool dx_fused_supported(int mode, int nb, int ng);
int dx_fused_lanes(dangx_ctx* ctx, const GroupArgs& ga, const IndexArgs& a, int Sp);
bool dx_launch_fused(dangx_ctx* ctx, const GroupArgs& ga, const IndexArgs& a, int Sp, int lanes, unsigned nblk, unsigned long long* accp);
int dx_mh_reg_lanes(int nb, int Sp);
int dx_planeset_lanes(dangx_ctx* ctx, const GroupArgs& ga, const SweepList& sl, int solve);
bool dx_launch_planeset(dangx_ctx* ctx, const GroupArgs& ga, const SweepList& sl, int lanes, int solve, unsigned nblk, unsigned long long* accp);
bool dx_launch_mh_reg(dangx_ctx* ctx, const IndexArgs& a, int Sp, unsigned nblk, unsigned long long* accp);
```

### dang_amd/csrc/dx_kern_fused.h

```cpp
#pragma once
#include "dx_chain.h"

struct FusedArgs {
    signed char vslot[MAXG];
    signed char vcomp[MAXG];
    signed char vtype[MAXG];
    int nv;
    int gself;
    int cal;
};

#ifndef DX_FUSED_WAVES
#define DX_FUSED_WAVES(SP, NB) 2
#endif
#ifndef DX_FUSED_GRP
#define DX_FUSED_GRP 5
#endif
namespace dxk {

template <int NBL>
__device__ __forceinline__ void sed_column(int type, const double* __restrict__ tab, int NB, int NG, int g, int jb, const Prep& p,
                                           double* __restrict__ colg) {
    const double* lnr = tab + (TROWS * g) * NB + jb;
    const double* cst = lnr + NB;
    const double* lnu9 = cst + NB;
    const double* nuc = tab + (TROWS * NG) * NB + jb;
    constexpr int TT = (NBL % 5 == 0) ? 5 : (NBL % 4 == 0) ? 4 : (NBL % 3 == 0) ? 3 : 1;
    if (type == DANGX_POWERLAW) {
#pragma unroll 1
        for (int j0 = 0; j0 < NBL; j0 += TT) {
#pragma unroll
            for (int t = 0; t < TT; ++t) colg[(j0 + t) * BLOCK] = exp_nr(p.p0 * lnr[j0 + t]);
        }
    } else if (type == DANGX_MBB) {
#pragma unroll 1
        for (int j0 = 0; j0 < NBL; j0 += TT) {
            double f[TT];
#pragma unroll
            for (int t = 0; t < TT; ++t) f[t] = p.p2 * fast_rcp(exp_nr(p.p1 * nuc[j0 + t]) - 1.0);
            __builtin_amdgcn_sched_barrier(0);
#pragma unroll
            for (int t = 0; t < TT; ++t) colg[(j0 + t) * BLOCK] = f[t] * exp_nr(p.p0 * lnr[j0 + t]);
        }
    } else if (type == DANGX_FREEFREE) {
        const double rp1 = fast_rcp(p.p1);
#pragma unroll 1
        for (int j0 = 0; j0 < NBL; j0 += TT) {
#pragma unroll
            for (int t = 0; t < TT; ++t) colg[(j0 + t) * BLOCK] = (ff_gaunt(lnu9[j0 + t], p.p0) * rp1) * cst[j0 + t];
        }
    } else {
        const double rp1 = fast_rcp(p.p1);
#pragma unroll 1
        for (int j0 = 0; j0 < NBL; j0 += TT) {
#pragma unroll
            for (int t = 0; t < TT; ++t) {
                const double l = (lnu9[j0 + t] - p.p2) * rp1;
                colg[(j0 + t) * BLOCK] = exp_sat(-0.5 * (l * l)) * cst[j0 + t];
            }
        }
    }
}

template <int NBL>
__device__ __forceinline__ void sed_column_bp(const Model& M, const Comp& c2, const double* __restrict__ tab, int NB, int NG, int g,
                                              const Prep& p, double* __restrict__ colg) {
#pragma unroll 1
    for (int j = 0; j < NBL; ++j) colg[j * BLOCK] = (M.band[j].n != 0) ? sed_bandpass(M, c2, j, p) : sed_eval_tab(c2.type, tab, NB, NG, g, j, p);
}

template <int MODE, int SP, int NB, int NG, int LP>
__global__ __launch_bounds__(BLOCK, DX_FUSED_WAVES(SP, NB)) void k_amp_index(const Model* __restrict__ Mp, GroupArgs ga, FusedArgs fa, IndexArgs a,
                                                                                  unsigned long long* __restrict__ not_spd,
                                                                                  unsigned long long* __restrict__ accepted,
                                                                                  double* __restrict__ chi_partial) {
    constexpr int NBL = NB / LP;
    extern __shared__ double lds[];
    const Model& M = *Mp;
    const int npix = M.npix, tid = threadIdx.x;
    double* tab = lds;
    double* col = lds + (TROWS * NG + 3) * NB + tid;
    const long long t0 = (long long)blockIdx.x * BLOCK + tid;
    const long long u = t0 / LP;
    const int half = (int)(t0 % LP), jb = half * NBL;
    const bool in_range = u < npix;
    const int i = in_range ? (int)u : 0;
    const double mk = M.mask[i];
    sed_table_build(M, tab, tid, BLOCK, ga.gc, NG);
    __syncthreads();
    double chi[4] = {0.0, 0.0, 0.0, 0.0};
    unsigned long long nacc = 0ull;
    const Comp& c = M.comp[a.comp];
    const bool live = in_range && !is_masked(mk);
    if (in_range && !live && half == 0) {
        double* out = c.idx + ((long long)a.nind * M.nmaps) * npix + i;
#pragma unroll
        for (int kk = 0; kk < SP; ++kk) out[(long long)(a.s1 + kk - 1) * npix] = 0.0;
    }
    if (live) {
        const BandPick<LP> pick = {half};
        RegChain<MODE, SP, NBL, LP> R;
        R.set_k(M, c, pick);
        const long long bstride = (long long)M.nmaps * npix;
        const unsigned long long gpix = (unsigned long long)(M.pix0 + i);
        const bool sample = (ga.ml_mode == DANGX_ML_SAMPLE);
#pragma unroll
        for (int kk = 0; kk < SP; ++kk) {
            const int k = a.s1 + kk;
            {
                const double* sigp = M.sig + (long long)(k - 1) * npix + i;
                const double* rmsp = M.rms + (long long)(k - 1) * npix + i;
#pragma unroll
                for (int j = 0; j < NBL; ++j) { R.D[kk][j] = sigp[(jb + j) * bstride]; R.ISr[kk][j] = rmsp[(jb + j) * bstride]; }
            }
            bool fresh = (kk == 0);
            double th0[NG], th1[NG];
#pragma unroll
            for (int v = 0; v < NG; ++v) {
                th0[v] = th1[v] = 0.0;
                if (v < fa.nv) load_theta(M, M.comp[ga.gc[fa.vcomp[v]]], i, k, th0[v], th1[v]);
            }
            if (kk > 0) {
#pragma unroll
                for (int v = 0; v < NG; ++v)
                    if (v < fa.nv) fresh = fresh || !(th0[v] == col[(fa.nv * NBL + 2 * v) * BLOCK] && th1[v] == col[(fa.nv * NBL + 2 * v + 1) * BLOCK]);
            }
            if (fresh) {
#pragma unroll
                for (int v = 0; v < NG; ++v)
                    if (v < fa.nv) { col[(fa.nv * NBL + 2 * v) * BLOCK] = th0[v]; col[(fa.nv * NBL + 2 * v + 1) * BLOCK] = th1[v]; }
#pragma unroll 1
                for (int v = 0; v < fa.nv; ++v) {
                    const Comp& c2 = M.comp[ga.gc[fa.vcomp[v]]];
                    const Prep pr = sed_prep(c2, col[(fa.nv * NBL + 2 * v) * BLOCK], col[(fa.nv * NBL + 2 * v + 1) * BLOCK]);
                    sed_column<NBL>(fa.vtype[v], tab, NB, NG, fa.vcomp[v], jb, pr, col + (v * NBL) * BLOCK);
                }
            }
            double eta = 0.0, f0 = 0.0;
            if (sample) {
                double u1, u2;
                uniform2(ga.seed, ga.stream, gpix, (uint32_t)k, u1, u2);
                eta = rand_normal(0.0, 1.0, u1, u2);
            }
            double A[NG * (NG + 1) / 2], bv[NG];
#pragma unroll
            for (int q = 0; q < NG * (NG + 1) / 2; ++q) A[q] = 0.0;
#pragma unroll
            for (int g = 0; g < NG; ++g) bv[g] = 0.0;
            const double* mp[NG];
            int ms[NG];
#pragma unroll
            for (int g = 0; g < NG; ++g) {
                const bool var = fa.vslot[g] >= 0;
                mp[g] = var ? col + (fa.vslot[g] * NBL) * BLOCK : tab + (TROWS * g + 2 + k) * NB + jb;
                ms[g] = var ? BLOCK : 1;
            }
#pragma unroll
            for (int j = 0; j < NBL; ++j) {
                double d = R.D[kk][j];
                if (SP == 1 && fa.cal) d = d / tab[(TROWS * NG + 1) * NB + jb + j];
                const double is = fast_rcp(R.ISr[kk][j]);
                R.set_is(kk, j, is);
                const double inv = is * is;
                double mrow[NG];
#pragma unroll
                for (int g = 0; g < NG; ++g) mrow[g] = mp[g][j * ms[g]];
#pragma unroll
                for (int g = 0; g < NG; ++g) {
                    const double t2 = mrow[g] * inv;
                    bv[g] += d * t2;
#pragma unroll
                    for (int h = 0; h <= g; ++h) A[g * (g + 1) / 2 + h] += t2 * mrow[h];
                }
                f0 += (eta * is) * mrow[NG - 1];
                if (j % DX_FUSED_GRP == DX_FUSED_GRP - 1) __builtin_amdgcn_sched_barrier(0);
            }
            if (LP > 1) {
#pragma unroll
                for (int q = 0; q < NG * (NG + 1) / 2; ++q) A[q] += __shfl_xor(A[q], 1, 64);
#pragma unroll
                for (int g = 0; g < NG; ++g) bv[g] += __shfl_xor(bv[g], 1, 64);
                f0 += __shfl_xor(f0, 1, 64);
            }
            bv[0] += f0;
            bool ok = true;
            double ri[NG];
#pragma unroll
            for (int g = 0; g < NG; ++g) {
#pragma unroll
                for (int h = 0; h <= g; ++h) {
                    double s = A[g * (g + 1) / 2 + h];
#pragma unroll
                    for (int t = 0; t < h; ++t) s -= A[g * (g + 1) / 2 + t] * A[h * (h + 1) / 2 + t];
                    if (h == g) {
                        if (!(s > 0.0) || !(s < 1.0e300)) ok = false;
                        ri[g] = fast_rsqrt(s);
                    } else {
                        A[g * (g + 1) / 2 + h] = s * ri[h];
                    }
                }
            }
            if (ok) {
#pragma unroll
                for (int g = 0; g < NG; ++g) {
                    double s = bv[g];
#pragma unroll
                    for (int t = 0; t < g; ++t) s -= A[g * (g + 1) / 2 + t] * bv[t];
                    bv[g] = s * ri[g];
                }
#pragma unroll
                for (int g = NG - 1; g >= 0; --g) {
                    double s = bv[g];
#pragma unroll
                    for (int t = g + 1; t < NG; ++t) s -= A[t * (t + 1) / 2 + g] * bv[t];
                    bv[g] = s * ri[g];
                }
                if (half == 0) {
#pragma unroll
                    for (int g = 0; g < NG; ++g) M.comp[ga.gc[g]].amp[(long long)(k - 1) * npix + i] = bv[g];
                }
            } else {
                if (half == 0) atomicAdd(not_spd, 1ull);
#pragma unroll
                for (int g = 0; g < NG; ++g) bv[g] = M.comp[ga.gc[g]].amp[(long long)(k - 1) * npix + i];
            }
            if (SP == 1 && fa.cal) {
                const double* gn = tab + (TROWS * NG + 1) * NB + jb;
#pragma unroll
                for (int j = 0; j < NBL; ++j) R.D[kk][j] = (R.D[kk][j] - gn[NB + j]) / gn[j];
            }
            R.amp[kk] = 0.0;
#pragma unroll
            for (int g = 0; g < NG; ++g) {
                if (g == fa.gself) { R.amp[kk] = bv[g]; continue; }
                if (!((a.others >> ga.gc[g]) & 1u)) continue;
                const double amp2 = bv[g];
                int ms2 = ms[g];
                if (SP == 2) asm volatile("" : "+s"(ms2));
#pragma unroll
                for (int j = 0; j < NBL; ++j) R.D[kk][j] -= amp2 * mp[g][j * ms2];
                __builtin_amdgcn_sched_barrier(0);
            }
        }
        double sample0, sample1;
        load_theta(M, c, i, a.s1, sample0, sample1);
        nacc = chain_finish<MODE, SP, NBL, LP>(M, a, c, R, pick, sample0, sample1, i, half, chi);
    }
    if (accepted) {
        for (int o = 32; o > 0; o >>= 1) nacc += __shfl_down(nacc, o, 64);
        if ((tid & 63) == 0 && nacc) atomicAdd(accepted, nacc);
    }
    if (chi_partial) {
        __shared__ double sh[4][BLOCK / 64];
#pragma unroll
        for (int q = 0; q < 4; ++q) {
            double v = chi[q];
            for (int o = 32; o > 0; o >>= 1) v += __shfl_down(v, o, 64);
            if ((tid & 63) == 0) sh[q][tid >> 6] = v;
        }
        __syncthreads();
        if (tid < 4) {
            double s = 0.0;
            for (int w = 0; w < BLOCK / 64; ++w) s += sh[tid][w];
            chi_partial[(long long)tid * gridDim.x + blockIdx.x] = s;
        }
    }
}

}
```

### dang_amd/csrc/dx_kern_planeset.h

```cpp
#pragma once
#include "dx_kern_fused.h"

#ifndef DX_PS_WAVES
#define DX_PS_WAVES(SP, NB, LP, SOLVE, C0) (((NB) / (LP) <= 5) ? 3 : 2)
#endif

namespace dxk {

template <int V> struct ItemCode { static constexpr int value = V; };
template <bool V> struct ItemFlag { static constexpr bool value = V; };

template <int MODE, int PAIR, int SP, int NBL, int LP, int NG, bool FIRST, bool LAST, bool BP, typename RFirst>
__device__ __forceinline__ void ps_item(const Model& M, const SweepList& sl, const SweepItem& it, RFirst& R0, int i, int half,
                                        int jb, int NB, const double* __restrict__ tab, const double* __restrict__ col,
                                        double& sample0, double& sample1, double chi_first[4],
                                        double chi_last[4], unsigned int* __restrict__ accepted, int slot, const double* first_acc) {
    const Comp& c = M.comp[it.comp];
    const BandPick<LP> pick = {half};
    const int npix = M.npix;
    IndexArgs a;
    a.comp = it.comp; a.nind = it.nind; a.s1 = sl.s1; a.s2 = sl.s2; a.nsample = sl.nsample; a.ml_mode = sl.ml_mode; a.mode = MODE;
    a.bp = 0; a.others = 0u; a.seed = sl.seed; a.stream = it.stream;
    RegChain<MODE, SP, NBL, LP, true, BP> R;
    R.set_kt(tab, NB, NG, it.gmember, jb);
#pragma unroll
    for (int kk = 0; kk < SP; ++kk) {
        R.amp[kk] = c.amp[(long long)(sl.s1 + kk - 1) * npix + i];
#pragma unroll
        for (int j = 0; j < NBL; ++j) { R.D[kk][j] = R0.D[kk][j]; R.ISr[kk][j] = col[(kk * NBL + j) * BLOCK] * R.amp[kk]; }
    }
    double chia[4] = {0.0, 0.0, 0.0, 0.0}, va, acc[2];
    unsigned long long na = chain_finish<MODE, SP, NBL, LP, false, !FIRST, (!PAIR && !LAST)>(M, a, c, R, pick, sample0, sample1, i, half, chia, &va,
                                                                                            FIRST ? first_acc : nullptr, acc);
    if (it.nind == 0) sample0 = va; else sample1 = va;
    if (FIRST) { chi_first[0] = chia[0]; chi_first[1] = chia[1]; }
    chi_last[2] = chia[2]; chi_last[3] = chia[3];
    unsigned long long nb_ = 0ull;
    if (PAIR) {
        constexpr int MODEB = (MODE == CH_MBB_BETA || MODE == CH_LOGN_NUP) ? MODE + 1 : MODE;
        RegChain<MODEB, SP, NBL, LP, true, BP> RB;
        RB.set_kt(tab, NB, NG, it.gmember, jb);
#pragma unroll
        for (int kk = 0; kk < SP; ++kk) {
            RB.amp[kk] = R.amp[kk];
#pragma unroll
            for (int j = 0; j < NBL; ++j) { RB.D[kk][j] = R.D[kk][j]; RB.ISr[kk][j] = R.ISr[kk][j]; }
        }
        IndexArgs b = a;
        b.nind = it.nind + 1; b.stream = it.stream2; b.mode = MODEB;
        double chib[4] = {0.0, 0.0, 0.0, 0.0}, vb;
        nb_ = chain_finish<MODEB, SP, NBL, LP, false, false, !LAST>(M, b, c, RB, pick, sample0, sample1, i, half, chib, &vb, acc);
        if (b.nind == 0) sample0 = vb; else sample1 = vb;
        chi_last[2] = chib[2]; chi_last[3] = chib[3];
        if (!LAST) {
#pragma unroll
            for (int kk = 0; kk < SP; ++kk)
#pragma unroll
                for (int j = 0; j < NBL; ++j) R0.D[kk][j] = RB.D[kk][j];
        }
    } else if (!LAST) {
#pragma unroll
        for (int kk = 0; kk < SP; ++kk)
#pragma unroll
            for (int j = 0; j < NBL; ++j) R0.D[kk][j] = R.D[kk][j];
    }
    if (accepted) {
        const int copy = threadIdx.x & 15;
        if (na) atomicAdd(accepted + (slot << 4) + copy, (unsigned int)na);
        if (nb_) atomicAdd(accepted + ((slot + 1) << 4) + copy, (unsigned int)nb_);
    }
}

template <int SP, int NB, int NG, int LP, int SOLVE, int C0, int C1, int C2, int C3, int BP = 0>
__global__ __launch_bounds__(BLOCK, DX_PS_WAVES(SP, NB, LP, SOLVE, C0)) void k_plane_set(const Model* __restrict__ Mp, GroupArgs ga, FusedArgs fa, SweepList sl,
                                                        unsigned long long* __restrict__ not_spd, unsigned long long* __restrict__ accepted,
                                                        double* __restrict__ chi_partial) {
    constexpr int NBL = NB / LP;
    extern __shared__ double lds[];
    const Model& M = *Mp;
    const int npix = M.npix, tid = threadIdx.x;
    double* tab = lds;
    double* col = lds + (TROWS * NG + 3) * NB + tid;
    const long long t0 = (long long)blockIdx.x * BLOCK + tid;
    const long long u = t0 / LP;
    const int half = (int)(t0 % LP), jb = half * NBL;
    const bool in_range = u < npix;
    const int i = in_range ? (int)u : 0;
    const double mk = M.mask[i];
    sed_table_build(M, tab, tid, BLOCK, ga.gc, NG);
    __shared__ unsigned int acc_blk[DX_MAX_IDXSUM * 16];
    if (tid < DX_MAX_IDXSUM * 16) acc_blk[tid] = 0u;
    __syncthreads();
    double chi[4] = {0.0, 0.0, 0.0, 0.0};
    constexpr int NS0 = C0 ? 1 + (C0 >> 3) : 0, NS1 = C1 ? 1 + (C1 >> 3) : 0, NS2 = C2 ? 1 + (C2 >> 3) : 0, NS3 = C3 ? 1 + (C3 >> 3) : 0;
    constexpr int NS = NS0 + NS1 + NS2 + NS3;
    const bool live = in_range && !is_masked(mk);
    if (in_range && !live && half == 0) {
        for (int q = 0; q < sl.n; ++q) {
            const Comp& c = M.comp[sl.s[q].comp];
            for (int e = 0; e <= sl.s[q].pair; ++e) {
                double* out = c.idx + ((long long)(sl.s[q].nind + e) * M.nmaps) * npix + i;
#pragma unroll
                for (int kk = 0; kk < SP; ++kk) out[(long long)(sl.s1 + kk - 1) * npix] = 0.0;
            }
        }
    }
    if (live) {
        const long long bstride = (long long)M.nmaps * npix;
        const unsigned long long gpix = (unsigned long long)(M.pix0 + i);
        const bool sample = (ga.ml_mode == DANGX_ML_SAMPLE);
#pragma unroll 1
        for (int v = 0; v < fa.nv; ++v) {
            const Comp& c2 = M.comp[ga.gc[fa.vcomp[v]]];
            double t0v, t1v;
            load_theta(M, c2, i, sl.s1, t0v, t1v);
            if (BP) sed_column_bp<NBL>(M, c2, tab, NB, NG, fa.vcomp[v], sed_prep(c2, t0v, t1v), col + (v * NBL) * BLOCK);
            else sed_column<NBL>(fa.vtype[v], tab, NB, NG, fa.vcomp[v], jb, sed_prep(c2, t0v, t1v), col + (v * NBL) * BLOCK);
        }
        RegChain<CH_POW, SP, NBL, LP> R0;
#pragma unroll
        for (int kk = 0; kk < SP; ++kk) {
            const int k = sl.s1 + kk;
            {
                const double* sigp = M.sig + (long long)(k - 1) * npix + i;
                const double* rmsp = M.rms + (long long)(k - 1) * npix + i;
#pragma unroll
                for (int j = 0; j < NBL; ++j) { R0.D[kk][j] = sigp[(jb + j) * bstride]; R0.ISr[kk][j] = rmsp[(jb + j) * bstride]; }
            }
            auto cal_transform = [&]() {
                const double* gn = tab + (TROWS * NG + 1) * NB + jb;
#pragma unroll
                for (int j = 0; j < NBL; ++j) R0.D[kk][j] = (R0.D[kk][j] - gn[NB + j]) / gn[j];
            };
            if (!SOLVE && SP == 1 && fa.cal) cal_transform();
#pragma unroll 1
            for (int t = 0; t < ga.nuc; ++t) {
                const Comp& ct = M.comp[ga.uc[t]];
                const double tv = ct.tmpl[(long long)(k - 1) * npix + i];
#pragma unroll
                for (int j = 0; j < NBL; ++j) R0.D[kk][j] -= ct.tamp[k - 1][jb + j] * tv;
            }
            double bv[NG];
            if (SOLVE) {
                double eta = 0.0, f0 = 0.0;
                if (sample) {
                    double u1, u2;
                    uniform2(ga.seed, ga.stream, gpix, (uint32_t)k, u1, u2);
                    eta = rand_normal(0.0, 1.0, u1, u2);
                }
                double A[NG * (NG + 1) / 2];
#pragma unroll
                for (int q = 0; q < NG * (NG + 1) / 2; ++q) A[q] = 0.0;
#pragma unroll
                for (int g = 0; g < NG; ++g) bv[g] = 0.0;
                const double* mp[NG];
                int ms[NG];
#pragma unroll
                for (int g = 0; g < NG; ++g) {
                    const bool var = fa.vslot[g] >= 0;
                    mp[g] = var ? col + (fa.vslot[g] * NBL) * BLOCK : tab + (TROWS * g + 2 + k) * NB + jb;
                    ms[g] = var ? BLOCK : 1;
                }
#pragma unroll
                for (int j = 0; j < NBL; ++j) {
                    double d = R0.D[kk][j];
                    if (SP == 1 && fa.cal) d = d / tab[(TROWS * NG + 1) * NB + jb + j];
                    const double is = fast_rcp(R0.ISr[kk][j]);
                    R0.set_is(kk, j, is);
                    const double inv = is * is;
                    double mrow[NG];
#pragma unroll
                    for (int g = 0; g < NG; ++g) mrow[g] = mp[g][j * ms[g]];
#pragma unroll
                    for (int g = 0; g < NG; ++g) {
                        const double t2 = mrow[g] * inv;
                        bv[g] += d * t2;
#pragma unroll
                        for (int h = 0; h <= g; ++h) A[g * (g + 1) / 2 + h] += t2 * mrow[h];
                    }
                    f0 += (eta * is) * mrow[NG - 1];
                    if (j % DX_FUSED_GRP == DX_FUSED_GRP - 1) __builtin_amdgcn_sched_barrier(0);
                }
                if (LP > 1) {
#pragma unroll
                    for (int q = 0; q < NG * (NG + 1) / 2; ++q) A[q] += __shfl_xor(A[q], 1, 64);
#pragma unroll
                    for (int g = 0; g < NG; ++g) bv[g] += __shfl_xor(bv[g], 1, 64);
                    f0 += __shfl_xor(f0, 1, 64);
                }
                bv[0] += f0;
                bool ok = true;
                double ri[NG];
#pragma unroll
                for (int g = 0; g < NG; ++g) {
#pragma unroll
                    for (int h = 0; h <= g; ++h) {
                        double s = A[g * (g + 1) / 2 + h];
#pragma unroll
                        for (int t = 0; t < h; ++t) s -= A[g * (g + 1) / 2 + t] * A[h * (h + 1) / 2 + t];
                        if (h == g) {
                            if (!(s > 0.0) || !(s < 1.0e300)) ok = false;
                            ri[g] = fast_rsqrt(s);
                        } else {
                            A[g * (g + 1) / 2 + h] = s * ri[h];
                        }
                    }
                }
                if (ok) {
#pragma unroll
                    for (int g = 0; g < NG; ++g) {
                        double s = bv[g];
#pragma unroll
                        for (int t = 0; t < g; ++t) s -= A[g * (g + 1) / 2 + t] * bv[t];
                        bv[g] = s * ri[g];
                    }
#pragma unroll
                    for (int g = NG - 1; g >= 0; --g) {
                        double s = bv[g];
#pragma unroll
                        for (int t = g + 1; t < NG; ++t) s -= A[t * (t + 1) / 2 + g] * bv[t];
                        bv[g] = s * ri[g];
                    }
#pragma unroll
                    for (int g = 0; g < NG; ++g) M.comp[ga.gc[g]].amp[(long long)(k - 1) * npix + i] = bv[g];
                } else {
                    if (half == 0) atomicAdd(not_spd, 1ull);
#pragma unroll
                    for (int g = 0; g < NG; ++g) bv[g] = M.comp[ga.gc[g]].amp[(long long)(k - 1) * npix + i];
                }
            } else {
#pragma unroll
                for (int g = 0; g < NG; ++g) bv[g] = M.comp[ga.gc[g]].amp[(long long)(k - 1) * npix + i];
#pragma unroll
                for (int j = 0; j < NBL; ++j) R0.set_is(kk, j, fast_rcp(R0.ISr[kk][j]));
            }
            if (SOLVE && SP == 1 && fa.cal) cal_transform();
#pragma unroll
            for (int g = 0; g < NG; ++g) {
                const double amp2 = bv[g];
                if (fa.vslot[g] >= 0) {
                    const double* m = col + (fa.vslot[g] * NBL) * BLOCK;
#pragma unroll
                    for (int j = 0; j < NBL; ++j) R0.D[kk][j] -= amp2 * m[j * BLOCK];
                } else {
                    const double* m = tab + (TROWS * g + 2 + k) * NB + jb;
#pragma unroll
                    for (int j = 0; j < NBL; ++j) R0.D[kk][j] -= amp2 * m[j];
                }
            }
#pragma unroll
            for (int j = 0; j < NBL; ++j) {
                R0.D[kk][j] *= R0.ISr[kk][j];
                asm volatile("" : "+v"(R0.D[kk][j]));
            }
        }
        double first_acc[2] = {0.0, 0.0};
        if (C0 == 0) {
#pragma unroll
            for (int kk = 0; kk < SP; ++kk) {
                double acc = 0.0;
#pragma unroll
                for (int j = 0; j < NBL; ++j) acc = fma(R0.D[kk][j], R0.D[kk][j], acc);
                if (LP > 1) acc += __shfl_xor(acc, 1, 64);
                if (half == 0) { chi[kk] = acc; chi[2 + kk] = acc; }
            }
        } else {
            {
                const SweepItem it0 = sl.s[0];
                const double* m = col + (fa.vslot[it0.gmember] * NBL) * BLOCK;
#pragma unroll
                for (int kk = 0; kk < SP; ++kk) {
                    const double a0 = M.comp[it0.comp].amp[(long long)(sl.s1 + kk - 1) * npix + i];
                    double acc = 0.0;
#pragma unroll
                    for (int j = 0; j < NBL; ++j) {
                        const double r = R0.D[kk][j];
                        acc = fma(r, r, acc);
                        R0.D[kk][j] = fma(a0 * R0.ISr[kk][j], m[j * BLOCK], r);
                    }
                    if (LP > 1) acc += __shfl_xor(acc, 1, 64);
                    first_acc[kk] = -0.5 * acc;
                }
            }
#pragma unroll
            for (int kk = 0; kk < SP; ++kk)
#pragma unroll
                for (int j = 0; j < NBL; ++j) col[(kk * NBL + j) * BLOCK] = R0.ISr[kk][j];
            __builtin_amdgcn_sched_barrier(0);
        }
        int slot = 0;
        auto run = [&](auto code_tag, auto first_tag, auto last_tag, int q) {
            constexpr int CODE = decltype(code_tag)::value;
            constexpr bool FIRST = decltype(first_tag)::value;
            constexpr bool LAST = decltype(last_tag)::value;
            if constexpr (CODE != 0) {
                const SweepItem it = sl.s[q];
                const Comp& c = M.comp[it.comp];
                double sample0, sample1, unused[4];
                load_theta(M, c, i, sl.s1, sample0, sample1);
                ps_item<(CODE & 7), (CODE >> 3), SP, NBL, LP, NG, FIRST, LAST, (BP != 0)>(M, sl, it, R0, i, half, jb, NB, tab, col, sample0, sample1,
                                                                              FIRST ? chi : unused, chi, accepted ? acc_blk : nullptr, slot, first_acc);
                slot += 1 + (CODE >> 3);
            }
        };
        run(ItemCode<C0>{}, ItemFlag<true>{}, ItemFlag<C1 == 0>{}, 0);
        run(ItemCode<C1>{}, ItemFlag<false>{}, ItemFlag<C2 == 0>{}, 1);
        run(ItemCode<C2>{}, ItemFlag<false>{}, ItemFlag<C3 == 0>{}, 2);
        run(ItemCode<C3>{}, ItemFlag<false>{}, ItemFlag<true>{}, 3);
    }
    if (accepted && NS > 0) {
        __syncthreads();
        if (tid < NS) {
            unsigned int v = 0u;
            for (int q = 0; q < 16; ++q) v += acc_blk[(tid << 4) + q];
            if (v != 0u) atomicAdd(accepted + tid, (unsigned long long)v);
        }
    }
    if (chi_partial) {
        double isum[NS > 0 ? NS : 1];
#pragma unroll
        for (int q = 0; q < (NS > 0 ? NS : 1); ++q) isum[q] = 0.0;
        if (live && half == 0) {
            constexpr int code[4] = {C0, C1, C2, C3};
            constexpr int first[4] = {0, NS0, NS0 + NS1, NS0 + NS1 + NS2};
#pragma unroll
            for (int q = 0; q < 4; ++q)
                if (code[q] != 0) {
                    const double* at = M.comp[sl.s[q].comp].idx + ((long long)sl.s[q].nind * M.nmaps + (sl.s1 - 1)) * npix + i;
                    isum[first[q]] = at[0];
                    if ((code[q] >> 3) != 0) isum[first[q] + 1] = at[(long long)M.nmaps * npix];
                }
        }
        __shared__ double sh[4 + NS][BLOCK / 64];
#pragma unroll
        for (int q = 0; q < 4 + NS; ++q) {
            double v = (q < 4) ? chi[q < 4 ? q : 0] : isum[q >= 4 ? q - 4 : 0];
            for (int o = 32; o > 0; o >>= 1) v += __shfl_down(v, o, 64);
            if ((tid & 63) == 0) sh[q][tid >> 6] = v;
        }
        __syncthreads();
        if (tid < 4 + NS) {
            double s = 0.0;
            for (int w = 0; w < BLOCK / 64; ++w) s += sh[tid][w];
            chi_partial[(long long)tid * gridDim.x + blockIdx.x] = s;
        }
    }
}

}
```

### include/dangx.h

```cpp
#ifndef DANGX_H
#define DANGX_H

#include <stdint.h>

#ifdef __cplusplus
extern "C" {
#endif

#define DANGX_MAX_BANDS 32
#define DANGX_MAX_COMPS 16
#define DANGX_MAX_IND 2
#define DANGX_MAX_GROUP 8

enum { DANGX_POWERLAW = 1, DANGX_MBB = 2, DANGX_FREEFREE = 3, DANGX_LOGNORMAL = 4, DANGX_CMB = 5, DANGX_TCMB = 6,
       DANGX_TEMPLATE = 7, DANGX_MONOPOLE = 8, DANGX_HIFIT = 9 };
enum { DANGX_LNL_CHISQ = 1, DANGX_LNL_MARGINAL = 2, DANGX_LNL_PRIOR = 3 };
enum { DANGX_PRIOR_GAUSSIAN = 1, DANGX_PRIOR_UNIFORM = 2, DANGX_PRIOR_JEFFREYS = 3 };
enum { DANGX_ML_SAMPLE = 1, DANGX_ML_OPTIMIZE = 2 };
enum { DANGX_FLAG_T = 1, DANGX_FLAG_Q = 2, DANGX_FLAG_U = 4, DANGX_FLAG_QU = 8 };
enum { DANGX_SOLVER_DIRECT = 0, DANGX_SOLVER_CG = 1 };
enum { DANGX_FLUCT_CORRECT = 0, DANGX_FLUCT_REFERENCE = 1 };
enum { DANGX_COARSE_REFERENCE = 0, DANGX_COARSE_DEGRADED = 1 };

enum {
    DANGX_K_AMP_DIRECT = 0, DANGX_K_INDEX_MH = 1, DANGX_K_SKY_CHISQ = 2, DANGX_K_REDUCE = 3,
    DANGX_K_CG_AX = 4, DANGX_K_CG_VEC = 5, DANGX_K_AMP_INDEX = 6, DANGX_K_MOMENTS = 7, DANGX_K_COUNT = 8
};

typedef struct dangx_ctx dangx_ctx;

typedef struct {
    int32_t npix;
    int32_t nmaps;
    int32_t nbands;
    int32_t ncomp;
    int64_t pix0;
    int64_t npix_global;
    int32_t device;
    int32_t reserved;
} dangx_dims;

typedef struct {
    int32_t type;
    int32_t is_synch;
    int32_t nindices;
    int32_t cg_group;
    int32_t sample_amplitude;
    int32_t reserved;
    double nu_ref;
    int32_t lnl_type[DANGX_MAX_IND];
    int32_t prior_type[DANGX_MAX_IND];
    double gauss_prior[DANGX_MAX_IND][2];
    double uni_prior[DANGX_MAX_IND][2];
    double step_size[DANGX_MAX_IND];
} dangx_comp_desc;

int dangx_create(dangx_ctx **ctx, const dangx_dims *dims);
int dangx_destroy(dangx_ctx *ctx);
const char *dangx_last_error(const dangx_ctx *ctx);
const char *dangx_version(void);
int dangx_set_stream(dangx_ctx *ctx, void *hip_stream);
typedef int (*dangx_allreduce_fn)(void *user, double *buf, int64_t n);
int dangx_set_allreduce(dangx_ctx *ctx, dangx_allreduce_fn fn, void *user, int is_root);
int dangx_synchronize(dangx_ctx *ctx);
int dangx_device_count(int *n);
int dangx_set_host_stride(dangx_ctx *ctx, int64_t plane_stride);

int dangx_set_band(dangx_ctx *ctx, int band, double nu_c_hz, int n, const double *nu0, const double *tau0);
int dangx_set_component(dangx_ctx *ctx, int comp , const dangx_comp_desc *desc);
int dangx_set_tcmb(dangx_ctx *ctx, double T_cmb);
int dangx_set_calibration(dangx_ctx *ctx, const double *gain, const double *offset);

enum { DANGX_A2T = 0, DANGX_A2F = 1, DANGX_F2T = 2 };
int dangx_unit_conversion(dangx_ctx *ctx, int band, int which, double *out);
int dangx_normalize_bandpass(const double *tau_in, int n, double *tau_out);
enum { DANGX_UNIT_UK_RJ = 0, DANGX_UNIT_UK_CMB = 1, DANGX_UNIT_MJY_SR = 2 };
int dangx_convert_maps(dangx_ctx *ctx, const int32_t *unit, const int32_t *cg_map, double *conversion);

int dangx_upload_data(dangx_ctx *ctx, const double *sig, const double *rms, const double *mask);
int dangx_adopt_device_data(dangx_ctx *ctx, const double *sig_dev, const double *rms_dev, const double *mask_dev);
int dangx_put_amplitude(dangx_ctx *ctx, int comp, const double *amp);
int dangx_get_amplitude(dangx_ctx *ctx, int comp, double *amp);
int dangx_put_indices(dangx_ctx *ctx, int comp, const double *ind);
int dangx_get_indices(dangx_ctx *ctx, int comp, double *ind);
int dangx_set_template(dangx_ctx *ctx, int comp, const double *tmpl, const int32_t *corr, int nfit);
int dangx_put_template_amplitudes(dangx_ctx *ctx, int comp, const double *ta);
int dangx_get_template_amplitudes(dangx_ctx *ctx, int comp, double *ta);
int dangx_adopt_device_state(dangx_ctx *ctx, int comp, double *amp_dev, double *idx_dev);
void *dangx_amplitude_devptr(dangx_ctx *ctx, int comp);
void *dangx_indices_devptr(dangx_ctx *ctx, int comp);

int dangx_amp_sample(dangx_ctx *ctx, int group, int flag, int ml_mode, int solver, int fluct_mode,
                     uint64_t seed, uint64_t stream, int i_max, double converge,
                     int *cg_iters, int64_t *n_not_spd);

int dangx_schur_info(dangx_ctx *ctx, double *rel_residual , int *refinements);
int dangx_amp_residual(dangx_ctx *ctx, int group, int flag, int ml_mode, uint64_t seed, uint64_t stream, double *out);

int dangx_index_sample(dangx_ctx *ctx, int comp, int nind, int map_n, int nsample, int ml_mode,
                       uint64_t seed, uint64_t stream, int64_t *accepted);

int dangx_index_sample_pair(dangx_ctx *ctx, int comp, int nind, int map_n, int nsample, int ml_mode, uint64_t seed,
                            uint64_t stream_first, uint64_t stream_second, int64_t *accepted_first, int64_t *accepted_second);

int dangx_amp_index_sample(dangx_ctx *ctx, int group, int flag, int ml_mode, int solver, int fluct_mode, uint64_t seed_amp,
                           uint64_t stream_amp, int i_max, double converge, int comp, int nind, int map_n, int nsample,
                           uint64_t seed_index, uint64_t stream_index, int *cg_iters, int64_t *n_not_spd, int64_t *accepted);

int dangx_plane_set_sample(dangx_ctx *ctx, int group, int flag, int ml_mode, int solver, int fluct_mode, uint64_t seed_amp,
                           uint64_t stream_amp, int i_max, double converge, int nsweeps, const int32_t *comp, const int32_t *nind,
                           const uint64_t *stream, int nsample, uint64_t seed_index, int *cg_iters, int64_t *n_not_spd,
                           int64_t *accepted);

int dangx_plane_sweeps_sample(dangx_ctx *ctx, int flag, int nsweeps, const int32_t *comp, const int32_t *nind, const uint64_t *stream,
                              int nsample, int ml_mode, uint64_t seed, int64_t *accepted);

int dangx_sky_model_chisq(dangx_ctx *ctx, int pol_lo, int pol_hi, double *chisq_sum,
                          double *sky, double *res, double *chi_map);
int dangx_sky_model_chisq_dev(dangx_ctx *ctx, int pol_lo, int pol_hi, double *chisq_sum_dev);

int dangx_chisq_cached(dangx_ctx *ctx, int which, int pol_lo, int pol_hi, double *chisq_sum);
int dangx_chisq_cached_dev(dangx_ctx *ctx, int which, int pol_lo, int pol_hi, double *chisq_sum_dev);

int dangx_chisq_current(dangx_ctx *ctx, int pol_lo, int pol_hi, double *chisq_sum);

int dangx_index_sample_coarse(dangx_ctx *ctx, int comp, int nind, int map_n, int nsample, int ml_mode,
                              uint64_t seed, uint64_t stream, int nside, int sample_nside, int64_t *accepted);
int dangx_coarse_sizes(dangx_ctx *ctx, int map_n, int sample_nside, int64_t *n_partials, int64_t *n_index);
int dangx_coarse_partials(dangx_ctx *ctx, int comp, int map_n, int nside, int sample_nside, double *buf);
int dangx_coarse_chains(dangx_ctx *ctx, int comp, int nind, int map_n, int nsample, int ml_mode, uint64_t seed, uint64_t stream,
                        int nside, int sample_nside, const double *partials_sum, double *index_out);
int dangx_coarse_writeback(dangx_ctx *ctx, int comp, int nind, int map_n, int nside, int sample_nside, const double *index_sum);
int dangx_set_coarse_model(dangx_ctx *ctx, int comp, int nind, int model);
int dangx_coarse_model_size(dangx_ctx *ctx, int comp, int map_n, int sample_nside, int64_t *n_model);
int dangx_coarse_model_partials(dangx_ctx *ctx, int comp, int map_n, int nside, int sample_nside, double *buf);
int dangx_coarse_model_finish(dangx_ctx *ctx, int comp, int map_n, int nside, int sample_nside, const double *model_sum);
int dangx_udgrade(dangx_ctx *ctx, int mode, const double *map_in, int nside_in, double *map_out, int nside_out);

int dangx_index_masked_sum(dangx_ctx *ctx, int comp, int nind, int map_n, double *sum, int64_t *count);

int dangx_index_masked_sums(dangx_ctx *ctx, int n, const int32_t *comp, const int32_t *nind, const int32_t *map_n, double *sums,
                            int64_t *counts);

int dangx_index_plain_sum(dangx_ctx *ctx, int comp, int nind, int map_n, double *sum_index, double *sum_mask);

int dangx_fullsky_prepare(dangx_ctx *ctx, int comp, int map_n);
int dangx_fullsky_prepare_coarse(dangx_ctx *ctx, int comp, int map_n, int nside, int sample_nside);
int dangx_fullsky_sums(dangx_ctx *ctx, int what, const double *theta, double *out, int nout);
int dangx_fill_index(dangx_ctx *ctx, int comp, int nind, int map_n, double value);
int dangx_gain_sums(dangx_ctx *ctx, int band, double *out);
int dangx_peek_indices(dangx_ctx *ctx, int comp, int map_n, long long pix, double *out);

int dangx_fullsky_finish_coarse(dangx_ctx *ctx, int comp, int map_n, int nside, int sample_nside, const double *partials_sum);

int dangx_fullsky_sample(dangx_ctx *const *ctxs, int nctx, int comp, int nind, int map_n, int nsample, int ml_mode,
                         uint64_t seed, uint64_t stream, int nside, int sample_nside, int32_t *tuned, double *step_size,
                         double *value, int64_t *accepted);
int dangx_tune_step_size(dangx_ctx *const *ctxs, int nctx, int comp, int nind, int nsample, int ml_mode, uint64_t seed,
                         uint64_t stream, const double *theta_init, uint32_t *draw, int32_t *tuned, double *step_size);
int dangx_tune_perpixel(dangx_ctx *const *ctxs, int nctx, int comp, int nind, int map_n, int nsample, int ml_mode,
                        uint64_t seed, uint64_t stream, int32_t *tuned, double *step_size);
int dangx_fit_band_gain(dangx_ctx *const *ctxs, int nctx, int band, int ml_mode, uint64_t seed, uint64_t stream, double *gain);
int dangx_update_tcmb(dangx_ctx *const *ctxs, int nctx, int comp, double *tcmb);

int dangx_plan_fusion(dangx_ctx *ctx, int npairs, const int32_t *pair_group, const int32_t *pair_flag, int nsweeps,
                      const int32_t *sweep_comp, const int32_t *sweep_nind, const int32_t *sweep_flag, const int32_t *sweep_plain,
                      int solver, int32_t *first_sweep);

int dangx_sky_amp_sample(dangx_ctx *const *ctxs, int nctx, int group, int flag, int ml_mode, int solver, int fluct_mode,
                         uint64_t seed, uint64_t stream, int i_max, double converge, int *cg_iters, int64_t *n_not_spd);

int dangx_sky_plane_set_sample(dangx_ctx *const *ctxs, int nctx, int group, int flag, int ml_mode, int solver, int fluct_mode,
                               uint64_t seed_amp, uint64_t stream_amp, int i_max, double converge, int nsweeps, const int32_t *comp,
                               const int32_t *nind, const uint64_t *stream, int nsample, uint64_t seed_index, int *cg_iters,
                               int64_t *n_not_spd, int64_t *accepted);

int64_t dangx_group_size(dangx_ctx *ctx, int group, int flag);
int dangx_compute_rhs(dangx_ctx *ctx, int group, int flag, double *b);
int dangx_compute_Ax(dangx_ctx *ctx, int group, int flag, const double *x, double *res);
int dangx_compute_sample_vector(dangx_ctx *ctx, int group, int flag, const double *eta, double *res);
int dangx_eval_sed(dangx_ctx *ctx, int comp, int band, int map_n, double *out);

int dangx_rtc_kernels(dangx_ctx *ctx, int *n, char *names, int names_len);
int dangx_rtc_compile(const char *header, const char *name_expr, char *log, int log_len);

int dangx_moments_begin(dangx_ctx *ctx, const int32_t *sel);
int dangx_moments_accumulate(dangx_ctx *ctx);
int dangx_moments_count(dangx_ctx *ctx, int64_t *n);
int dangx_moments_get(dangx_ctx *ctx, int comp, int what, int stat, int ddof, double *out);
int dangx_moments_get_dev(dangx_ctx *ctx, int comp, int what, int stat, int ddof, double *out_dev);
int dangx_moments_get_template(dangx_ctx *ctx, int comp, int stat, int ddof, double *ta);
int dangx_moments_end(dangx_ctx *ctx);

int dangx_profile_enable(dangx_ctx *ctx, int on);
int dangx_profile_reset(dangx_ctx *ctx);
int dangx_profile_get(dangx_ctx *ctx, int kernel_id, double *total_ms, int64_t *launches);
int dangx_profile_get_planes(dangx_ctx *ctx, int kernel_id, int nplanes, double *total_ms, int64_t *launches);

#ifdef __cplusplus
}
#endif
#endif
```

Before: 98.51.

## Reuse precomputed SED columns and MBB factors across planeset sweep items

Adds three reuse paths to the planeset kernel, enabled by default through DX_PS_REUSE=7. Later sweep items take their likelihood from the SED column already staged in LDS instead of recomputing it. The MBB frequency factors written during sed_column are kept in an extra LDS row and reused when an MBB beta item finishes. In paired MBB chains the exponentials from the beta certification pass are passed on to the temperature step. The varying-component slots are reordered so the columns match the sweep order. This trades extra LDS use (which could lower occupancy) and more template variants for fewer exp and divide evaluations. A budget query API is also exposed.

```diff
diff --git a/dang_amd/_lib.py b/dang_amd/_lib.py
--- a/dang_amd/_lib.py
+++ b/dang_amd/_lib.py
@@ -135,6 +135,7 @@
     "dangx_eval_sed": (C.c_int, [_P, C.c_int, C.c_int, C.c_int, _P]),
     "dangx_rtc_kernels": (C.c_int, [_P, C.POINTER(C.c_int), C.c_char_p, C.c_int]),
     "dangx_rtc_compile": (C.c_int, [C.c_char_p, C.c_char_p, C.c_char_p, C.c_int]),
+    "dangx_planeset_budget": (C.c_int, [C.c_int, C.c_int, C.c_int, C.c_int, C.c_int, _P]),
     "dangx_moments_begin": (C.c_int, [_P, _P]),
     "dangx_moments_accumulate": (C.c_int, [_P]),
     "dangx_moments_count": (C.c_int, [_P, C.POINTER(C.c_int64)]),
diff --git a/dang_amd/csrc/dangx_fused.hip b/dang_amd/csrc/dangx_fused.hip
--- a/dang_amd/csrc/dangx_fused.hip
+++ b/dang_amd/csrc/dangx_fused.hip
@@ -54,7 +54,7 @@
 }
 
 static bool fused_args(dangx_ctx* ctx, const GroupArgs& ga, const IndexArgs& a, FusedArgs& fa) {
-    fa.nv = 0; fa.gself = -1;
+    fa.nv = 0; fa.gself = -1; fa.frow = -1; fa.fslot = -1;
     unsigned planes = 0;
     for (int k = a.s1; k <= a.s2; ++k) planes |= 1u << (k - 1);
     for (int g = 0; g < MAXG; ++g) { fa.vslot[g] = -1; fa.vcomp[g] = 0; fa.vtype[g] = 0; }
diff --git a/dang_amd/csrc/dangx_planeset.hip b/dang_amd/csrc/dangx_planeset.hip
--- a/dang_amd/csrc/dangx_planeset.hip
+++ b/dang_amd/csrc/dangx_planeset.hip
@@ -8,6 +8,26 @@
     const int rows = nv > Sp ? nv : Sp;
     return ((size_t)(TROWS * ng + 3) * nb + (size_t)rows * (nb / lanes) * BLOCK) * sizeof(double);
 }
+
+static constexpr int PS_CAP1 = 16, PS_CAP2 = 13;
+
+static int planeset_shape_lanes(int ng, int nb, int nv, int Sp, bool small_too, int cap) {
+    if (small_too && nb <= cap && planeset_lds(ng, nb, nv, 1, Sp) <= 80u * 1024u) return 1;
+    if (nb > 12 && nb % 2 == 0 && nb / 2 <= cap && planeset_lds(ng, nb, nv, 2, Sp) <= 80u * 1024u) return 2;
+    return 0;
+}
+
+static size_t planeset_lds_rows(int ng, int nb, int nv, int lanes, int Sp, bool want_planck, int* frow) {
+    const size_t base = planeset_lds(ng, nb, nv, lanes, Sp);
+    const size_t budget = (nb / lanes <= 5) ? (160u * 1024u) / 3u : 80u * 1024u;
+    const size_t with = base + (size_t)(nb / lanes) * BLOCK * sizeof(double);
+    *frow = -1;
+    if (!(DX_PS_REUSE & 2) || !want_planck || lanes == 2 || with > budget) return base;
+    *frow = (nv > Sp ? nv : Sp) * (nb / lanes);
+    return with;
+}
+
+int dx_planeset_reuse() { return DX_PS_REUSE; }
 
 static void item_codes(const SweepList& sl, int code[4]) {
     for (int q = 0; q < 4; ++q) code[q] = (q < sl.n) ? sl.s[q].mode + 8 * sl.s[q].pair : 0;
@@ -47,7 +67,7 @@
 }
 
 static bool planeset_args(dangx_ctx* ctx, const GroupArgs& ga, const SweepList& sl, FusedArgs& fa) {
-    fa.nv = 0; fa.gself = -1;
+    fa.nv = 0; fa.gself = -1; fa.frow = -1; fa.fslot = -1;
     unsigned planes = 0;
     for (int k = sl.s1; k <= sl.s2; ++k) planes |= 1u << (k - 1);
     for (int g = 0; g < MAXG; ++g) { fa.vslot[g] = -1; fa.vcomp[g] = 0; fa.vtype[g] = 0; }
@@ -63,6 +83,21 @@
             fa.vslot[g] = (signed char)fa.nv++;
         }
     }
+    if ((DX_PS_REUSE & 1) && sl.n > 0 && fa.nv > 1) {
+        int order[MAXG], no = 0;
+        auto swept_at = [&](int g) { for (int q = 0; q < sl.n; ++q) if (sl.s[q].gmember == g) return q; return -1; };
+        for (int v = 0; v < fa.nv; ++v) if (swept_at(fa.vcomp[v]) == 0) order[no++] = fa.vcomp[v];
+        for (int v = 0; v < fa.nv; ++v) if (swept_at(fa.vcomp[v]) < 0) order[no++] = fa.vcomp[v];
+        for (int q = 1; q < sl.n; ++q)
+            for (int v = 0; v < fa.nv; ++v) if (swept_at(fa.vcomp[v]) == q) order[no++] = fa.vcomp[v];
+        for (int v = 0; v < no; ++v) {
+            fa.vcomp[v] = (signed char)order[v]; fa.vtype[v] = (signed char)ctx->hm.comp[ga.gc[order[v]]].type;
+            fa.vslot[order[v]] = (signed char)v;
+        }
+    }
+    for (int q = 0; q < sl.n && fa.fslot < 0; ++q)
+        if (sl.s[q].mode == CH_MBB_BETA && sl.s[q].gmember >= 0 && sl.s[q].gmember < ga.ng && fa.vslot[sl.s[q].gmember] >= 0 &&
+            ctx->hm.comp[ga.gc[sl.s[q].gmember]].type == DANGX_MBB) fa.fslot = fa.vslot[sl.s[q].gmember];
     fa.cal = 0;
     if (sl.s1 == 1)
         for (int j = 0; j < ctx->hm.nbands; ++j)
@@ -74,8 +109,8 @@
     static const bool enabled = [] { const char* e = getenv("DANGX_PLANESET"); return !(e && e[0] == '0'); }();
     static const bool small_too = [] { const char* e = getenv("DANGX_PLANESET"); return !(e && e[0] == 'p'); }();
     if (!enabled || sl.n < 0 || sl.n > 4 || (sl.n == 0 && !solve) || ga.ng < 1 || ga.ng > 6) return 0;
-    static const int cap2 = [] { const char* e = getenv("DANGX_PS_CAP2"); return e ? atoi(e) : 13; }();
-    const int nb = ctx->hm.nbands, Sp = sl.s2 - sl.s1 + 1, cap = (Sp == 2) ? cap2 : 16;
+    static const int cap2 = [] { const char* e = getenv("DANGX_PS_CAP2"); return e ? atoi(e) : PS_CAP2; }();
+    const int nb = ctx->hm.nbands, Sp = sl.s2 - sl.s1 + 1, cap = (Sp == 2) ? cap2 : PS_CAP1;
     for (int q = 0; q < sl.n; ++q) {
         const int m = sl.s[q].mode;
         if (m < CH_POW || m > CH_LOGN_W) return 0;
@@ -91,9 +126,7 @@
         if (!(small_too && nb <= cap && planeset_lds(ga.ng, nb, fa.nv, 1, Sp) <= 80u * 1024u)) return 0;
         return dx_rtc_get(ctx, "dx_kern_planeset.h", planeset_name(Sp, nb, ga.ng, 1, solve, sl, 1)) ? 1 : 0;
     }
-    int lanes = 0;
-    if (small_too && nb <= cap && planeset_lds(ga.ng, nb, fa.nv, 1, Sp) <= 80u * 1024u) lanes = 1;
-    else if (nb > 12 && nb % 2 == 0 && nb / 2 <= cap && planeset_lds(ga.ng, nb, fa.nv, 2, Sp) <= 80u * 1024u) lanes = 2;
+    const int lanes = planeset_shape_lanes(ga.ng, nb, fa.nv, Sp, small_too, cap);
     if (!lanes) return 0;
     if (planeset_builtin(nb, ga.ng, lanes, solve, sl)) return lanes;
     return dx_rtc_get(ctx, "dx_kern_planeset.h", planeset_name(Sp, nb, ga.ng, lanes, solve, sl, 0)) ? lanes : 0;
@@ -103,8 +136,8 @@
     FusedArgs fa;
     if (lanes < 1 || lanes > 2 || !planeset_args(ctx, ga, sl, fa)) return false;
     const int nb = ctx->hm.nbands, ng = ga.ng, Sp = sl.s2 - sl.s1 + 1;
-    const size_t ldsz = planeset_lds(ng, nb, fa.nv, lanes, Sp);
     const int bp = planeset_bp(ctx);
+    const size_t ldsz = planeset_lds_rows(ng, nb, fa.nv, lanes, Sp, !bp && fa.fslot >= 0, &fa.frow);
     if (!bp && planeset_builtin(nb, ng, lanes, solve, sl)) {
         if (nb == 20) launch_builtin<20, 6, 2, 1, CH_POW, CH_MBB_BETA + 8, CH_LOGN_NUP>(ctx, ga, fa, sl, Sp, nblk, ldsz, accp);
         else if (nb == 10 && sl.n == 0) launch_builtin<10, 4, 1, 1, 0, 0, 0>(ctx, ga, fa, sl, Sp, nblk, ldsz, accp);
@@ -125,6 +158,18 @@
     return dx_rtc_launch(ctx, fn, nblk, ldsz, args) == 0;
 }
 
+extern "C" int dangx_planeset_budget(int nbands, int nmembers, int nvarying, int nplanes, int mbb_beta_item, int32_t* out) {
+    if (!out || nbands < 1 || nmembers < 1 || nmembers > MAXG || nvarying < 0 || nvarying > nmembers || nplanes < 1 || nplanes > 2) return 1;
+    const int lanes = planeset_shape_lanes(nmembers, nbands, nvarying, nplanes, true, nplanes == 2 ? PS_CAP2 : PS_CAP1);
+    out[0] = lanes; out[1] = out[2] = 0; out[3] = -1;
+    if (!lanes) return 0;
+    int frow = -1;
+    out[1] = (int32_t)planeset_lds(nmembers, nbands, nvarying, lanes, nplanes);
+    out[2] = (int32_t)planeset_lds_rows(nmembers, nbands, nvarying, lanes, nplanes, mbb_beta_item != 0, &frow);
+    out[3] = frow;
+    return 0;
+}
+
 #ifdef DX_LNL_DIAG
 extern "C" int dangx_lnl_diag(unsigned long long* out) {
     if (hipMemcpyFromSymbol(out, HIP_SYMBOL(g_lnl_diag), 2 * sizeof(unsigned long long)) != hipSuccess) return 1;
diff --git a/dang_amd/csrc/dangx_rtc.hip b/dang_amd/csrc/dangx_rtc.hip
--- a/dang_amd/csrc/dangx_rtc.hip
+++ b/dang_amd/csrc/dangx_rtc.hip
@@ -62,10 +62,14 @@
 std::vector<std::string> extra_options() {
     std::vector<std::string> out;
     const char* e = getenv("DANGX_RTC_DEFS");
-    if (!e) return out;
-    std::istringstream ss(e);
-    std::string w;
-    while (ss >> w) out.push_back(w);
+    if (e) {
+        std::istringstream ss(e);
+        std::string w;
+        while (ss >> w) out.push_back(w);
+    }
+    out.push_back("-UDX_PS_RECOMPUTE");
+    out.push_back("-UDX_PS_REUSE");
+    out.push_back("-DDX_PS_REUSE=" + std::to_string(dx_planeset_reuse()));
     return out;
 }
 
diff --git a/dang_amd/csrc/dx_chain.h b/dang_amd/csrc/dx_chain.h
--- a/dang_amd/csrc/dx_chain.h
+++ b/dang_amd/csrc/dx_chain.h
@@ -24,6 +24,18 @@
 #endif
 #ifndef DX_CHAIN_PAIR_RNG
 #define DX_CHAIN_PAIR_RNG 1
+#endif
+
+#if defined(DX_CHAIN_LIBEXP) || defined(DX_CHAIN_IEEEDIV) || defined(DX_CHAIN_UNSCALED)
+#undef DX_PS_REUSE
+#define DX_PS_REUSE 0
+#endif
+#ifndef DX_PS_REUSE
+#ifdef DX_PS_RECOMPUTE
+#define DX_PS_REUSE 0
+#else
+#define DX_PS_REUSE 7
+#endif
 #endif
 
 namespace {
@@ -105,8 +117,9 @@
         }
     }
 
-    template <bool BATCH, int OP = 0>
-    __device__ __forceinline__ double lnl(const Model& M, const Comp& c, double th, double other, double& acc0, double& acc1) {
+    template <bool BATCH, int OP = 0, bool EXPO = false>
+    __device__ __forceinline__ double lnl(const Model& M, const Comp& c, double th, double other, double& acc0, double& acc1,
+                                          double* eout = nullptr) {
         double s0 = 0.0, s1 = 0.0;
         if (MODE == CH_POW) s0 = th;
         else if (MODE == CH_MBB_BETA) s0 = th + 1.0;
@@ -169,6 +182,7 @@
                     s[t] = CEXPS(-0.5 * (l * l)) * k2(c, j);
                 } else {
                     const double e = CEXP(s0 * k1(M, c, j));
+                    if (EXPO) eout[j] = e;
                     if (MODE == CH_POW) s[t] = e;
                     else if (MODE == CH_MBB_BETA) s[t] = F[j] * e;
                     else s[t] = CDIV(s1, e - 1.0) * F[j];
@@ -224,6 +238,28 @@
         return acc0 + acc1;
     }
 
+    __device__ __forceinline__ double lnl_add_col(const double* __restrict__ scol, double& acc0, double& acc1) {
+        acc0 = 0.0; acc1 = 0.0;
+#pragma unroll
+        for (int j = 0; j < NB; ++j) {
+            const double s = scol[j * BLOCK];
+            const double r0 = D[0][j];
+            D[0][j] = fma(is(0, j), s, r0);
+            acc0 = fma(r0, r0, acc0);
+            if (SP == 2) {
+                const double r1 = D[SP - 1][j];
+                D[SP - 1][j] = fma(is(SP - 1, j), s, r1);
+                acc1 = fma(r1, r1, acc1);
+            }
+        }
+        if (LP > 1) {
+            acc0 += __shfl_xor(acc0, 1, 64);
+            if (SP == 2) acc1 += __shfl_xor(acc1, 1, 64);
+        }
+        acc0 *= -0.5; acc1 *= -0.5;
+        return acc0 + acc1;
+    }
+
     __device__ __forceinline__ double lnl_cheap(const Model& M, const Comp& c, double th) {
         double s0 = 0.0, s1 = 0.0;
         if (MODE == CH_POW) s0 = th;
@@ -364,24 +400,36 @@
     }
 }
 
-template <int MODE, int SP, int NB, int LP, bool SCALE = true, bool ADD = false, bool SUB = false, class RC>
+template <int MODE, int SP, int NB, int LP, bool SCALE = true, bool ADD = false, bool SUB = false, int COL = 0, class RC>
 __device__ __forceinline__ unsigned long long chain_finish(const Model& M, const IndexArgs& a, const Comp& c, RC& R,
                                                            const BandPick<LP>& pick, double sample0, double sample1, int i, int half,
                                                            double chi[4], double* final_value = nullptr,
-                                                           const double* acc_in = nullptr, double* acc_out = nullptr) {
+                                                           const double* acc_in = nullptr, double* acc_out = nullptr,
+                                                           const double* scol = nullptr, const double* frows = nullptr,
+                                                           double* fx = nullptr, bool* fx_ok = nullptr) {
     const int npix = M.npix;
     double* out = c.idx + ((long long)a.nind * M.nmaps) * npix + i;
     const bool first = (a.nind == 0);
     if (SCALE) R.scale();
     if (MODE == CH_MBB_BETA) {
-        const double z = mbb_z(sample1);
-        const double A = CEXP(z * c.nu_ref) - 1.0;
-#pragma unroll
-        for (int j = 0; j < NB; ++j) R.F[j] = CDIV(A, CEXP(z * pick.nu_c(M, j, NB)) - 1.0);
-        if (RC::kBP) { R.bpa = z; R.bpb = A; }
+        if (!RC::kBP && frows) {
+#pragma unroll
+            for (int j = 0; j < NB; ++j) R.F[j] = frows[j * BLOCK];
+        } else {
+            const double z = mbb_z(sample1);
+            const double A = CEXP(z * c.nu_ref) - 1.0;
+#pragma unroll
+            for (int j = 0; j < NB; ++j) R.F[j] = CDIV(A, CEXP(z * pick.nu_c(M, j, NB)) - 1.0);
+            if (RC::kBP) { R.bpa = z; R.bpb = A; }
+        }
     } else if (MODE == CH_MBB_T) {
-#pragma unroll
-        for (int j = 0; j < NB; ++j) R.F[j] = CEXP((sample0 + 1.0) * pick(c.lnr, j, NB));
+        if (!RC::kBP && fx && *fx_ok) {
+#pragma unroll
+            for (int j = 0; j < NB; ++j) R.F[j] = fx[j];
+        } else {
+#pragma unroll
+            for (int j = 0; j < NB; ++j) R.F[j] = CEXP((sample0 + 1.0) * pick(c.lnr, j, NB));
+        }
         if (RC::kBP) R.bpa = sample0 + 1.0;
     } else if (MODE == CH_LOGN_W) {
         {
@@ -419,6 +467,7 @@
         constexpr bool B = decltype(batch_tag)::value;
         double lnl;
         if (acc_in) { a0 = acc_in[0]; a1 = acc_in[1]; lnl = a0 + a1; }
+        else if (ADD && !RC::kBP && (COL == 1 || (COL == 2 && scol))) lnl = R.lnl_add_col(scol, a0, a1);
         else lnl = R.template lnl<B, ADD ? 1 : 0>(M, c, cur, other, a0, a1);
         chi[0] = -2.0 * a0; chi[1] = -2.0 * a1;
         double lnl_old = lnl + prior(cur);
@@ -498,6 +547,11 @@
             double s0_, s1_;
             (void)R.template lnl<B, 2>(M, c, cur, other, s0_, s1_);
             if (!sums_exact) { a0 = s0_; a1 = s1_; }
+        } else if (kCert && MODE == CH_MBB_BETA && fx && cert) {
+            double s0_, s1_;
+            (void)R.template lnl<B, 0, true>(M, c, cur, other, s0_, s1_, fx);
+            if (!sums_exact) { a0 = s0_; a1 = s1_; }
+            *fx_ok = true;
         } else if (kCert) {
             if (__builtin_amdgcn_ballot_w64(!sums_exact) != 0ull) {
                 if (!sums_exact) (void)R.template lnl<B>(M, c, cur, other, a0, a1);
diff --git a/dang_amd/csrc/dx_host.h b/dang_amd/csrc/dx_host.h
--- a/dang_amd/csrc/dx_host.h
+++ b/dang_amd/csrc/dx_host.h
@@ -264,4 +264,5 @@
 int dx_mh_reg_lanes(int nb, int Sp);
 int dx_planeset_lanes(dangx_ctx* ctx, const GroupArgs& ga, const SweepList& sl, int solve);
 bool dx_launch_planeset(dangx_ctx* ctx, const GroupArgs& ga, const SweepList& sl, int lanes, int solve, unsigned nblk, unsigned long long* accp);
+int dx_planeset_reuse();
 bool dx_launch_mh_reg(dangx_ctx* ctx, const IndexArgs& a, int Sp, unsigned nblk, unsigned long long* accp);
diff --git a/dang_amd/csrc/dx_kern_fused.h b/dang_amd/csrc/dx_kern_fused.h
--- a/dang_amd/csrc/dx_kern_fused.h
+++ b/dang_amd/csrc/dx_kern_fused.h
@@ -8,6 +8,8 @@
     int nv;
     int gself;
     int cal;
+    int frow;
+    int fslot;
 };
 
 #ifndef DX_FUSED_WAVES
@@ -20,7 +22,7 @@
 
 template <int NBL>
 __device__ __forceinline__ void sed_column(int type, const double* __restrict__ tab, int NB, int NG, int g, int jb, const Prep& p,
-                                           double* __restrict__ colg) {
+                                           double* __restrict__ colg, double* __restrict__ frows = nullptr) {
     const double* lnr = tab + (TROWS * g) * NB + jb;
     const double* cst = lnr + NB;
     const double* lnu9 = cst + NB;
@@ -39,6 +41,10 @@
 #pragma unroll
             for (int t = 0; t < TT; ++t) f[t] = p.p2 * fast_rcp(exp_nr(p.p1 * nuc[j0 + t]) - 1.0);
             __builtin_amdgcn_sched_barrier(0);
+            if (frows) {
+#pragma unroll
+                for (int t = 0; t < TT; ++t) frows[(j0 + t) * BLOCK] = f[t];
+            }
 #pragma unroll
             for (int t = 0; t < TT; ++t) colg[(j0 + t) * BLOCK] = f[t] * exp_nr(p.p0 * lnr[j0 + t]);
         }
diff --git a/dang_amd/csrc/dx_kern_planeset.h b/dang_amd/csrc/dx_kern_planeset.h
--- a/dang_amd/csrc/dx_kern_planeset.h
+++ b/dang_amd/csrc/dx_kern_planeset.h
@@ -11,7 +11,7 @@
 template <bool V> struct ItemFlag { static constexpr bool value = V; };
 
 template <int MODE, int PAIR, int SP, int NBL, int LP, int NG, bool FIRST, bool LAST, bool BP, typename RFirst>
-__device__ __forceinline__ void ps_item(const Model& M, const SweepList& sl, const SweepItem& it, RFirst& R0, int i, int half,
+__device__ __forceinline__ void ps_item(const Model& M, const FusedArgs& fa, const SweepList& sl, const SweepItem& it, RFirst& R0, int i, int half,
                                         int jb, int NB, const double* __restrict__ tab, const double* __restrict__ col,
                                         double& sample0, double& sample1, double chi_first[4],
                                         double chi_last[4], unsigned int* __restrict__ accepted, int slot, const double* first_acc) {
@@ -30,8 +30,17 @@
         for (int j = 0; j < NBL; ++j) { R.D[kk][j] = R0.D[kk][j]; R.ISr[kk][j] = col[(kk * NBL + j) * BLOCK] * R.amp[kk]; }
     }
     double chia[4] = {0.0, 0.0, 0.0, 0.0}, va, acc[2];
-    unsigned long long na = chain_finish<MODE, SP, NBL, LP, false, !FIRST, (!PAIR && !LAST)>(M, a, c, R, pick, sample0, sample1, i, half, chia, &va,
-                                                                                            FIRST ? first_acc : nullptr, acc);
+    constexpr int REUSE = (LP == 2) ? 0 : DX_PS_REUSE;
+    constexpr int COL = ((REUSE & 1) && !FIRST && !BP && MODE <= CH_MBB_T) ? (SP == 1 ? 1 : 2) : 0;
+    const int vs = fa.vslot[it.gmember];
+    const double* scol = (COL == 1 || (COL == 2 && vs >= SP)) ? col + (vs * NBL) * BLOCK : nullptr;
+    const double* frows = ((REUSE & 2) && !BP && MODE == CH_MBB_BETA && fa.frow >= 0 && fa.fslot == vs) ? col + fa.frow * BLOCK : nullptr;
+    constexpr bool FX = (REUSE & 4) && !BP && PAIR && MODE == CH_MBB_BETA;
+    double fxv[FX ? NBL : 1];
+    bool fx_ok = false;
+    unsigned long long na = chain_finish<MODE, SP, NBL, LP, false, !FIRST, (!PAIR && !LAST), COL>(M, a, c, R, pick, sample0, sample1, i, half, chia, &va,
+                                                                                                 FIRST ? first_acc : nullptr, acc, scol, frows,
+                                                                                                 FX ? fxv : nullptr, &fx_ok);
     if (it.nind == 0) sample0 = va; else sample1 = va;
     if (FIRST) { chi_first[0] = chia[0]; chi_first[1] = chia[1]; }
     chi_last[2] = chia[2]; chi_last[3] = chia[3];
@@ -49,7 +58,8 @@
         IndexArgs b = a;
         b.nind = it.nind + 1; b.stream = it.stream2; b.mode = MODEB;
         double chib[4] = {0.0, 0.0, 0.0, 0.0}, vb;
-        nb_ = chain_finish<MODEB, SP, NBL, LP, false, false, !LAST>(M, b, c, RB, pick, sample0, sample1, i, half, chib, &vb, acc);
+        nb_ = chain_finish<MODEB, SP, NBL, LP, false, false, !LAST>(M, b, c, RB, pick, sample0, sample1, i, half, chib, &vb, acc, nullptr, nullptr, nullptr,
+                                                                    FX ? fxv : nullptr, &fx_ok);
         if (b.nind == 0) sample0 = vb; else sample1 = vb;
         chi_last[2] = chib[2]; chi_last[3] = chib[3];
         if (!LAST) {
@@ -115,7 +125,8 @@
             double t0v, t1v;
             load_theta(M, c2, i, sl.s1, t0v, t1v);
             if (BP) sed_column_bp<NBL>(M, c2, tab, NB, NG, fa.vcomp[v], sed_prep(c2, t0v, t1v), col + (v * NBL) * BLOCK);
-            else sed_column<NBL>(fa.vtype[v], tab, NB, NG, fa.vcomp[v], jb, sed_prep(c2, t0v, t1v), col + (v * NBL) * BLOCK);
+            else sed_column<NBL>(fa.vtype[v], tab, NB, NG, fa.vcomp[v], jb, sed_prep(c2, t0v, t1v), col + (v * NBL) * BLOCK,
+                                 ((DX_PS_REUSE & 2) && LP != 2 && fa.frow >= 0 && fa.fslot == v) ? col + fa.frow * BLOCK : nullptr);
         }
         RegChain<CH_POW, SP, NBL, LP> R0;
 #pragma unroll
@@ -298,7 +309,7 @@
                 const Comp& c = M.comp[it.comp];
                 double sample0, sample1, unused[4];
                 load_theta(M, c, i, sl.s1, sample0, sample1);
-                ps_item<(CODE & 7), (CODE >> 3), SP, NBL, LP, NG, FIRST, LAST, (BP != 0)>(M, sl, it, R0, i, half, jb, NB, tab, col, sample0, sample1,
+                ps_item<(CODE & 7), (CODE >> 3), SP, NBL, LP, NG, FIRST, LAST, (BP != 0)>(M, fa, sl, it, R0, i, half, jb, NB, tab, col, sample0, sample1,
                                                                               FIRST ? chi : unused, chi, accepted ? acc_blk : nullptr, slot, first_acc);
                 slot += 1 + (CODE >> 3);
             }
diff --git a/include/dangx.h b/include/dangx.h
--- a/include/dangx.h
+++ b/include/dangx.h
@@ -184,6 +184,8 @@
 int dangx_rtc_kernels(dangx_ctx *ctx, int *n, char *names, int names_len);
 int dangx_rtc_compile(const char *header, const char *name_expr, char *log, int log_len);
 
+int dangx_planeset_budget(int nbands, int nmembers, int nvarying, int nplanes, int mbb_beta_item, int32_t *out);
+
 int dangx_moments_begin(dangx_ctx *ctx, const int32_t *sel);
 int dangx_moments_accumulate(dangx_ctx *ctx);
 int dangx_moments_count(dangx_ctx *ctx, int64_t *n);
```

Measured after the change: 100.6 (median of 6 runs). +2.2%, better.
